# DavidPeicho/cuda-pathtracer

Measured on AMD Instinct MI355X. Metric: Msamples/sec at 1920x1080, 4 spp, indoor.obj, higher is better.
Workload: dtype f32

## Files before the change

### cuda-pathtracer_amd/csrc/pt_device.h

```cpp
#pragma once

#include <hip/hip_runtime.h>
#include <stdint.h>

#include "pt_round.h"

namespace ptamd {

struct f3 { float x, y, z; };

#define PT_DEV __device__ __forceinline__
#define PT_HD __host__ __device__ __forceinline__

PT_HD f3 mk3(float x, float y, float z) { f3 r; r.x = x; r.y = y; r.z = z; return r; }
PT_HD f3 mk3(float s) { return mk3(s, s, s); }
PT_HD f3 operator+(f3 a, f3 b) { return mk3(a.x + b.x, a.y + b.y, a.z + b.z); }
PT_HD f3 operator+(f3 a, float b) { return mk3(a.x + b, a.y + b, a.z + b); }
PT_HD f3 operator-(f3 a, f3 b) { return mk3(a.x - b.x, a.y - b.y, a.z - b.z); }
PT_HD f3 operator-(f3 a, float b) { return mk3(a.x - b, a.y - b, a.z - b); }
PT_HD f3 operator-(f3 a) { return mk3(-a.x, -a.y, -a.z); }
PT_HD f3 operator*(f3 a, f3 b) { return mk3(a.x * b.x, a.y * b.y, a.z * b.z); }
PT_HD f3 operator*(f3 a, float b) { return mk3(a.x * b, a.y * b, a.z * b); }
PT_HD f3 operator*(float b, f3 a) { return mk3(b * a.x, b * a.y, b * a.z); }
PT_HD f3 operator/(f3 a, f3 b) { return mk3(a.x / b.x, a.y / b.y, a.z / b.z); }
// ... 286 lines not shown
  while (!miss_tail_is_closed(thr)) {
    if (miss_tail_iteration(env, max_bounces, acc, thr, bk, r1, rng, rcp)) return futile;
    ++futile;
  }
  const f3 e = env * thr;
  const uint32_t n = miss_tail_count(bk & 0xffffu, max_bounces);
  for (uint32_t i = 0; i < n; ++i) acc = acc + e;
  return futile + n - 1u;
}


struct TexDesc { int32_t w, h, nb_chan; uint32_t pad; uint64_t offset; };

#define PT_HEAD_STRIDE 64u
#ifndef PT_TILE_W_LOG2
#define PT_TILE_W_LOG2 3u
#endif
#define PT_TILE_W (1u << PT_TILE_W_LOG2)
#define PT_TILE_H (64u >> PT_TILE_W_LOG2)
struct KParams {
  const float4* nodes;
  const float4* tris_bvh;
  const float4* tris_brute;
  const float4* shade;
  const int4* materials;
  const float4* lights;
  const TexDesc* textures;
  const float* texels;
  const float4* cubemap;
  uint32_t cubemap_size;
  uint32_t n_faces, n_lights, n_nodes, n_bvh_tris;
  f3 cam_pos, cam_p0, cam_u, cam_v;
  float focus_dist, aperture;
  uint32_t width, height, row_begin, row_end;
  uint32_t hash_seed;
  float frame_nb_f;
  float frame_nb_inv;
  int32_t is_static;
  int32_t bounces;
  uint32_t post_id;
  float* tfb;
  uint32_t* surface;
  uint32_t tfb_row0;
  uint32_t tfb_reset;
  uint32_t surf_row0;
  unsigned long long* stats;
  unsigned long long* error_flag;
  union { uint32_t* tile_counter; uint32_t* adaptive; };
  uint32_t* tile_heads;
  uint32_t n_static;
  uint32_t tiles_x, n_tiles, tiles_per_ticket;
  uint32_t refill_min;
  uint32_t sample_count, frame_nb0;
  float* samples_out;
  float4* pool;
  uint32_t pool_lds_offset;
  uint32_t round_min, round_div;
  uint32_t round_div_m16;
  uint32_t walk_min;
  uint32_t small_det;
  uint32_t env_uniform;
  float env_r, env_g, env_b;
  const float* gamma_table;
  const float4* nodes4;
  uint32_t n_nodes4;
  uint32_t stack_lds_entries, stack_spill_entries;
  uint32_t ilv_ranks, ilv_rank, ilv_rows;
  uint32_t y_limit;
  uint32_t treelet_nodes;
  uint2* stack_spill;
  uint32_t walk_min4;
  uint32_t wide8;
  uint32_t far_table[16];
  uint32_t xcd_regions;
  uint32_t brute_walk;
  unsigned long long* timeline;
  uint32_t round_form;
  uint32_t round_defer;
};
#define PT_ROUND_GENERIC 1u
#define PT_ROUND_FLAT 2u
#define PT_ROUND_SKIP 4u
#define PT_ROUND_DEFER 8u
#define PT_SKIP_ENTRY_BYTES 32u

#define PT_RS_PLAIN 0
#define PT_RS_STATS 1
#define PT_RS_STAMPS 2
#define PT_RS_BRUTE 3
#define PT_RS_WIDE8 4
#define PT_RS_WIDE4Q 5
#define PT_RS_GENERIC 6
#define PT_RS_LIST 7
#define PT_RS_FLAT 8
#define PT_RS_FLAT_SKIP 9
#define PT_RS_PLAIN_SKIP 10
#define PT_RS_FLAT_SKIP_DEFER 11
#define PT_RS_PLAIN_SKIP_DEFER 12
#define PT_RS_STATS_DEFER 13
#define PT_RS_FORMS 14

struct RestartTraits {
  bool stats;
  bool stamps;
  bool brute;
  int wide;
  bool list;
  bool lean;
  bool flat;
  bool skip;
  bool defer;
  int reports;
  bool resident, streamed, contracted;
};
constexpr RestartTraits kRestartForms[] = {
  { false, false, false, 0, false, true,  false, false, false, PT_RS_PLAIN,      true,  true,  true },
  { true,  false, false, 0, false, false, false, false, false, PT_RS_STATS,      true,  true,  false },
  { false, true,  false, 0, false, false, false, false, false, PT_RS_STAMPS,     true,  true,  false },
  { false, false, true,  0, false, false, false, false, false, PT_RS_BRUTE,      true,  true,  true },
  { false, false, false, 1, false, false, false, false, false, PT_RS_WIDE8,      false, true,  false },
  { false, false, false, 2, false, false, false, false, false, PT_RS_WIDE4Q,     false, true,  false },
  { false, false, false, 0, false, false, false, false, false, PT_RS_GENERIC,    true,  false, true },
  { false, false, false, 0, true,  false, false, false, false, PT_RS_LIST,       true,  true,  false },
  { false, false, false, 0, false, true,  true,  false, false, PT_RS_FLAT,       true,  false, false },
  { false, false, false, 0, false, true,  true,  true,  false, PT_RS_FLAT_SKIP,  true,  false, false },
  { false, false, false, 0, false, true,  false, true,  false, PT_RS_PLAIN_SKIP, true,  false, false },
  { false, false, false, 0, false, true,  true,  true,  true,  PT_RS_FLAT_SKIP,  true,  false, false },
  { false, false, false, 0, false, true,  false, true,  true,  PT_RS_PLAIN_SKIP, true,  false, false },
  { true,  false, false, 0, false, false, false, false, true,  PT_RS_STATS,      true,  false, false },
};
static_assert(sizeof kRestartForms / sizeof kRestartForms[0] == PT_RS_FORMS, "one row per PT_RS_* number");
constexpr RestartTraits restart_traits(int variant) { return kRestartForms[variant]; }

inline bool restart_shipped_launch(const KParams& p)
{
  return p.is_static && p.pool_lds_offset && !p.xcd_regions && p.ilv_ranks <= 1u && !(p.round_form & PT_ROUND_GENERIC);
}

struct RestartForm { int variant; bool lds_resident; };
inline RestartForm restart_select(bool lds_resident, bool stats, bool list, bool contracted, const KParams* p)
{
  const auto full = [contracted](int variant) { return contracted ? PT_RS_PLAIN : variant; };
  if (list && !contracted) return { PT_RS_LIST, lds_resident };
  const bool defers = p && lds_resident && !contracted && (p->round_form & PT_ROUND_DEFER) && (p->round_form & PT_ROUND_SKIP) && !p->brute_walk && !p->timeline &&
                      restart_shipped_launch(*p);
  if (stats) return { defers ? PT_RS_STATS_DEFER : full(PT_RS_STATS), lds_resident };
  if (p && p->brute_walk) return { PT_RS_BRUTE, lds_resident };
  if (p && p->timeline) return { full(PT_RS_STAMPS), lds_resident };
  if (!lds_resident && p && p->wide8) return { full(p->wide8 == 2u ? PT_RS_WIDE4Q : PT_RS_WIDE8), false };
  if (!lds_resident) return { PT_RS_PLAIN, false };
  if (p && !restart_shipped_launch(*p)) return { PT_RS_GENERIC, true };
  if (defers) return { (p->round_form & PT_ROUND_FLAT) ? PT_RS_FLAT_SKIP_DEFER : PT_RS_PLAIN_SKIP_DEFER, true };
  if (p && (p->round_form & PT_ROUND_SKIP) && !contracted) return { (p->round_form & PT_ROUND_FLAT) ? PT_RS_FLAT_SKIP : PT_RS_PLAIN_SKIP, true };
  if (p && (p->round_form & PT_ROUND_FLAT)) return { full(PT_RS_FLAT), true };
  return { PT_RS_PLAIN, true };
}
#define PT_POOL_LDS_BYTES 2304u

struct Hit {
  f3 normal;
  f3 diffuse_col;
  float dist;
  float specular_col;
  float ior;
  int light;
  float emission;
};

}
```

### cuda-pathtracer_amd/csrc/pt_kernels.hip

```cpp
#include "pt_device.h"
#include "pt_launch.h"
#include "pt_adaptive.h"

#include <utility>

#ifndef PT_FMA_BUILD
#include "pt_denoise.h"
#endif

namespace ptamd {

#ifndef PT_TILE_THREADS
#define PT_TILE_THREADS 512
#endif
#ifndef PT_TILE_WAVES_PER_EU
#define PT_TILE_WAVES_PER_EU 6
#endif
#ifndef PT_SP_THREADS
#define PT_SP_THREADS 768
#endif
#ifndef PT_SP_SHADERS
#define PT_SP_SHADERS 7
#endif
#ifndef PT_SP_WAVES_PER_EU
#define PT_SP_WAVES_PER_EU 6
#endif
#ifndef PT_SP_FETCH_MIN
#define PT_SP_FETCH_MIN 16u
#endif
#ifndef PT_BW_THREADS
#define PT_BW_THREADS 512
#endif
#ifndef PT_BW_WAVES_PER_EU
#define PT_BW_WAVES_PER_EU 4
#endif
#ifndef PT_BW_FETCH_MIN
#define PT_BW_FETCH_MIN 16u
#endif
#ifndef PT_PERSISTENT_WAVES_PER_EU
#define PT_PERSISTENT_WAVES_PER_EU 6
#endif
#ifndef PT_PERSISTENT_THREADS
#define PT_PERSISTENT_THREADS 512
#endif
#ifndef PT_RS_THREADS
#define PT_RS_THREADS 768
#endif
#ifndef PT_RS_WAVES_PER_EU
#define PT_RS_WAVES_PER_EU 6
#endif
#ifndef PT_ASM_LEAF
#define PT_ASM_LEAF 1
#endif
#ifndef PT_WALK_PRIO
#define PT_WALK_PRIO 3
#endif
#define PT_STR2(x) #x
#define PT_STR(x) PT_STR2(x)
#define PT_MAX_DIST 100000.0f
#define PT_END 0xFFFFFFFFu


struct Best { float t, u, v; uint32_t idx; };

template <bool ORDERED>
PT_DEV void mt_test(float4 a, float4 b, float4 c, f3 o, f3 d, Best& best, bool small_det = false)
{
  const f3 e1 = mk3(a.x, a.y, a.z);
  const f3 e2 = mk3(a.w, b.x, b.y);
  const f3 v0 = mk3(b.z, b.w, c.x);
  const f3 p_vec = cross(d, e2);
  const float det = dot(e1, p_vec);
  if (det < 1e-7f) return;
  const float inv_det = small_det ? rcp_exact_in_range(det) : 1.0f / det;
  const f3 t_vec = o - v0;
  const float u = dot(t_vec, p_vec) * inv_det;
  if (u < 0 || u > 1) return;
  const f3 qvec = cross(t_vec, e1);
  const float v = dot(d, qvec) * inv_det;
  if (v < 0 || u + v > 1) return;
  const float t = dot(e2, qvec) * inv_det;
  const uint32_t idx = f_as_u(c.y);
  bool take;
  if (ORDERED) take = t < best.t && t > 0.0f;
  else take = t > 0.0f && (t < best.t || (t == best.t && idx < best.idx && best.idx != PT_END));
  if (take) { best.t = t; best.u = u; best.v = v; best.idx = idx; }
}

PT_DEV void mt_test_asm(float4 a, float4 b, float2 c, f3 o, f3 d, Best& best)
// ... 160 lines not shown
                                       __builtin_fmaxf(t0z, t1z));
    const bool hit = tnear <= tfar && tfar >= 0.0f && tnear <= w.best.t;
    const uint32_t info = f_as_u(q0.w);
    const uint32_t child = f_as_u(q1.w);
    const uint32_t count = info >> 24;
    const uint32_t down = ((w.oct >> (child >> 30)) & 1u) ? (child & 0x3FFFFFFFu) : node + 1u;
    node = (hit && count == 0u) ? down : miss;
    if (hit && count != 0u) {
      leaf_first = info & 0xFFFFFFu;
      leaf_count = count;
      break;
    }
    if (walk_min > 1u && (uint32_t)__popcll(__ballot(1)) < walk_min) break;
  }
  w.node = node;
}

static_assert(PT_TILE_WAVES_PER_EU <= 6 && PT_PERSISTENT_WAVES_PER_EU <= 6 && PT_RS_WAVES_PER_EU <= 6 && PT_SP_WAVES_PER_EU <= 6,
              "walk_to_leaf_lds_state clobbers v64..v74: kernels that inline it need a budget of at least 75 VGPRs (<= 6 waves per SIMD)");
PT_DEV void walk_to_leaf_lds_state(uint32_t& state, uint32_t lnk, const Walk& w, uint32_t& leaf_first, uint32_t& leaf_count, uint32_t walk_min)
{
  unsigned long long save;
  uint32_t link_word;
  uint32_t walkers;
  asm volatile(
      "s_mov_b64 %[save], exec\n\t"
      "s_setprio " PT_STR(PT_WALK_PRIO) "\n\t"
      "v_cmp_gt_u32 vcc, 0x8000, %[st]\n\t"
      "s_and_b64 exec, exec, vcc\n\t"
      "s_cbranch_execz 2f\n\t"
      "1:\n\t"
      "v_add_u32 v74, %[st], %[lnk]\n\t"
      "ds_read_b128 v[64:67], %[st]\n\t"
      "ds_read_b64 v[68:69], %[st] offset:16\n\t"
      "ds_read_b32 %[lw], v74\n\t"
      "s_waitcnt lgkmcnt(1)\n\t"
      "v_fma_f32 v64, v64, %[ix], %[nx]\n\t"
      "v_fma_f32 v65, v65, %[iy], %[ny]\n\t"
      "v_fma_f32 v66, v66, %[iz], %[nz]\n\t"
      "v_fma_f32 v74, -v67, |%[ix]|, v64\n\t"
      "v_fma_f32 v64, v67, |%[ix]|, v64\n\t"
      "v_fma_f32 v67, -v68, |%[iy]|, v65\n\t"
      "v_fma_f32 v65, v68, |%[iy]|, v65\n\t"
      "v_fma_f32 v68, -v69, |%[iz]|, v66 clamp\n\t"
      "v_fma_f32 v66, v69, |%[iz]|, v66\n\t"
      "v_max3_f32 v74, v74, v67, v68\n\t"
      "v_min3_f32 v64, v64, v65, v66\n\t"
      "v_min_f32 v64, v64, %[best]\n\t"
      "v_cmp_le_f32 vcc, v74, v64\n\t"
      "s_waitcnt lgkmcnt(0)\n\t"
      "s_nop 0\n\t"
      "v_cndmask_b32_sdwa %[st], %[lw], %[lw], vcc dst_sel:DWORD dst_unused:UNUSED_PAD src0_sel:WORD_1 src1_sel:WORD_0\n\t"
      "v_cmpx_gt_u32 vcc, 0x8000, %[st]\n\t"
      "s_bcnt1_i32_b64 %[walkers], exec\n\t"
      "s_cmp_ge_u32 %[walkers], %[wmin]\n\t"
      "s_cbranch_scc1 1b\n\t"
      "2:\n\t"
      "s_mov_b64 exec, %[save]\n\t"
      "s_setprio 0\n\t"
      : [st] "+v"(state), [lw] "=&v"(link_word), [save] "=&s"(save), [walkers] "=&s"(walkers)
      : [wmin] "s"(walk_min), [lnk] "v"(lnk), [ix] "v"(w.inv.x), [iy] "v"(w.inv.y), [iz] "v"(w.inv.z),
        [nx] "v"(w.noi.x), [ny] "v"(w.noi.y), [nz] "v"(w.noi.z), [best] "v"(w.best.t * PT_T_SCALE)
      : "v64", "v65", "v66", "v67", "v68", "v69", "v74", "vcc", "scc", "memory");
  leaf_first = 0u;
  leaf_count = 0u;
  if (state >= 0x8000u && state != 0xFFFFu) {
    leaf_first = state & 0x7FFu;
    leaf_count = (state >> 11) & 0xFu;
    state = link_word >> 16;
  }
}

PT_DEV uint32_t walk_lds_link_offset(const Walk& w) { return w.n_nodes * 32u + w.oct * 4u; }
PT_DEV uint32_t walk_lds_state(uint32_t lds_nodes, uint32_t node) { return node == PT_END ? 0xFFFFu : lds_nodes + (node << 5); }
PT_DEV uint32_t walk_lds_node(uint32_t lds_nodes, uint32_t state) { return state == 0xFFFFu ? PT_END : (state - lds_nodes) >> 5; }

PT_DEV void walk_to_leaf_lds(uint32_t lds_nodes, Walk& w, uint32_t& leaf_first, uint32_t& leaf_count, uint32_t walk_min = 1u)
{
  uint32_t state = walk_lds_state(lds_nodes, w.node);
  walk_to_leaf_lds_state(state, walk_lds_link_offset(w), w, leaf_first, leaf_count, walk_min);
  w.node = walk_lds_node(lds_nodes, state);
}

template <bool STATS, bool ASM = false>
PT_DEV void walk_leaf(const float4* tris, Walk& w, uint32_t leaf_first, uint32_t leaf_count, uint32_t& n_tris,
                      uint32_t& wave_tri_iters, bool small_det = false, uint32_t stride = 3u )
{
  if (ASM && !STATS && PT_ASM_LEAF && small_det) {
    for (uint32_t k = 0; k < leaf_count; ++k) {
      const float4* r = tris + (leaf_first + k) * stride;
      const float4 a = r[0], b = r[1];
      const float2 c = *reinterpret_cast<const float2*>(r + 2);
      mt_test_asm(a, b, c, w.o, w.d, w.best);
    }
    return;
  }
  for (uint32_t k = 0; k < leaf_count; ++k) {
    if (STATS) {
      const unsigned long long act = __ballot(1);
      if ((threadIdx.x & 63u) == (uint32_t)(__ffsll((long long)act) - 1)) ++wave_tri_iters;
    }
    const uint32_t ti = (leaf_first + k) * stride;
    mt_test<false>(tris[ti], tris[ti + 1], tris[ti + 2], w.o, w.d, w.best, small_det);
  }
  if (STATS) n_tris += leaf_count;
}

template <bool STATS, bool NODES_IN_LDS = false>
PT_DEV void traverse_bvh(const float4* nodes, const float4* tris, uint32_t n_nodes, f3 o, f3 d,
                         Best& best, uint32_t& n_nodes_visited, uint32_t& n_tris, uint32_t& wave_node_iters,
                         uint32_t& wave_tri_iters, uint32_t* idle3)
{
  Walk w;
  walk_init(w, o, d, n_nodes, NODES_IN_LDS && !STATS);
  if (STATS) w.alive = (uint32_t)__popcll(__ballot(1));
  const uint32_t lds_nodes = (uint32_t)(uintptr_t)nodes;
  for (;;) {
    uint32_t leaf_first, leaf_count;
    if (NODES_IN_LDS && !STATS) walk_to_leaf_lds(lds_nodes, w, leaf_first, leaf_count);
    else walk_to_leaf<STATS>(nodes, w, leaf_first, leaf_count, n_nodes_visited, wave_node_iters);
    if (leaf_count != 0u) walk_leaf<STATS>(tris, w, leaf_first, leaf_count, n_tris, wave_tri_iters);
    else if (w.node == PT_END) break;
  }
  best = w.best;
  if (STATS) { idle3[0] += w.idle_unstarted; idle3[1] += w.idle_finished; idle3[2] += w.idle_parked; }
}

PT_DEV bool intersect_sphere(f3 o, f3 d, f3 center, float radius2 , float& t)
{
  const float epsilon = 0.01f;
  const f3 op = center - o;
  const float b = dot(op, d);
  float disc = b * b - dot(op, op) + radius2;
  if (disc < 0.0f) return false;
  disc = sqrt_checked(disc);
  t = b - disc;
  if (!(t > epsilon)) t = b + disc;
  return t != 0.0f;
}

PT_DEV int texture_idx(const TexDesc& tex, float uvx, float uvy)
{
  int x = (int)(uvx * (float)(tex.w - 1));
  int y = (int)(uvy * (float)(tex.h - 1));
  return (y * tex.w + x) * tex.nb_chan;
}

struct Counters { uint32_t rays, nodes, tris, mesh_hits, nmap_hits, wave_node_iters, wave_tri_iters, fetch_events, fetch_rays, idle3[3];
                  unsigned long long cyc[16]; };
#define PT_WAVE_ONE() ((threadIdx.x & 63u) == (uint32_t)(__ffsll((long long)__ballot(1)) - 1))

struct Nearest { float t, u, v; uint32_t idx; };
#define PT_LIGHT 0x80000000u

typedef const __attribute__((address_space(4))) float* ConstF;
PT_DEV ConstF as_constant(const float4* q) { return (ConstF)(uintptr_t)q; }

#define PT_KERNEL_PARAMS const KParams p
template <typename T>
PT_DEV T karg_load(uint32_t byte_offset)
{
  const __attribute__((address_space(4))) char* q = (const __attribute__((address_space(4))) char*)__builtin_amdgcn_kernarg_segment_ptr();
  asm volatile("" : "+s"(q));
  return *(const __attribute__((address_space(4))) T*)(q + byte_offset);
}
#define PT_KARG(p, field) karg_load<decltype(KParams::field)>((uint32_t)__builtin_offsetof(KParams, field))

PT_DEV Nearest nearest_lights(const KParams& p, f3 o, f3 d, Nearest n)
{
  const ConstF lights = as_constant(p.lights);
  for (uint32_t l = 0; l < p.n_lights; ++l) {
    const ConstF L = lights + l * 8u;
    const f3 c = mk3(L[3], L[4], L[5]);
    const f3 op = c - o;
    const float b = dot(op, d);
    const float disc = b * b - dot(op, op) + L[7];
    if (__builtin_amdgcn_ballot_w64(!(disc < 0.0f)) == 0ull) continue;
// ... 297 lines not shown
        const float f_t = 1.0f - f_r;
        st.throughput = st.throughput * (f_t * direct_light);
        st.o = st.o + oriented_normal * inter.dist / 10000.f;
        st.d = T;
      }
    }
  }
  if (STATS) { asm volatile("" : "+v"(st.d.x), "+v"(st.o.x), "+v"(st.throughput.x)); const long long tp1 = clock64(); if (PT_WAVE_ONE()) cnt.cyc[11] += (unsigned long long)(tp1 - tp0); }
  const float pmax = __builtin_fmaxf(st.throughput.x, __builtin_fmaxf(st.throughput.y, st.throughput.z));
  if (r1 > pmax && st.b() > 1u) return true;
  st.throughput = st.throughput * rcp_hot(pmax);
  ++st.bk;
  return (int)st.b() >= max_bounces;
}




PT_DEV void stage_to_lds(float4* dst, const float4* src, uint32_t n16)
{
  for (uint32_t i = threadIdx.x; i < n16; i += blockDim.x) dst[i] = src[i];
}

template <int KIND, bool STATS, bool NODES_IN_LDS = false>
PT_DEV bool path_step(const KParams& p, const float4* s_nodes, const float4* s_tris, Path& st, Counters& cnt)
{
  const float r1 = path_pre(p, st);
  const Nearest n = trace_nearest<KIND, STATS, NODES_IN_LDS>(p, s_nodes, s_tris, st.o, st.d, cnt);
  return path_post<STATS>(p, st, r1, n, cnt);
}


PT_DEV void path_finish(const KParams& p, const Path& st)
{
  f3 rad = mk3(clamp01(st.acc.x), clamp01(st.acc.y), clamp01(st.acc.z));
  const uint32_t x = st.x(), y = st.y();
  const size_t i = (size_t)(p.height - y - 1u - p.tfb_row0) * p.width + x;
  float* tp = p.tfb + i * 3;
  f3 t = p.tfb_reset ? mk3(0.0f) : mk3(tp[0], tp[1], tp[2]);
  t = t * (float)p.is_static;
  t = t + rad;
  tp[0] = t.x; tp[1] = t.y; tp[2] = t.z;
  rad = p.frame_nb_inv != 0.0f ? t * p.frame_nb_inv : t / p.frame_nb_f;
  rad = exposure(rad);
  uint32_t px;
  if (p.gamma_table && p.post_id == 0u) {
    px = gamma_byte(rad.x, p.gamma_table) | (gamma_byte(rad.y, p.gamma_table) << 8) | (gamma_byte(rad.z, p.gamma_table) << 16);
  } else {
    const float g = 1.0f / 2.2f;
    rad = mk3(pt_powf(rad.x, g), pt_powf(rad.y, g), pt_powf(rad.z, g));
    rad = post_process(p.post_id, rad);
    px = (pt_f2u(rad.x * 255.0f) & 0xffu) | ((pt_f2u(rad.y * 255.0f) & 0xffu) << 8) | ((pt_f2u(rad.z * 255.0f) & 0xffu) << 16);
  }
  p.surface[(size_t)(y - p.surf_row0) * p.width + x] = px;
}

PT_DEV void path_finish_sample(const KParams& p, const Path& st)
{
  const uint32_t row_begin = PT_KARG(p, row_begin), rows = PT_KARG(p, row_end) - row_begin;
  float* sp = PT_KARG(p, samples_out) + (((size_t)st.k() * rows + (st.y() - row_begin)) * PT_KARG(p, width) + st.x()) * 3;
  sp[0] = clamp01(st.acc.x); sp[1] = clamp01(st.acc.y); sp[2] = clamp01(st.acc.z);
}

template <bool STATS>
PT_DEV void flush_counters(const KParams& p, const Counters& cnt, uint32_t samples)
{
  if (!STATS) return;
  const uint32_t lane = threadIdx.x & 63u;
  unsigned long long v[13] = { cnt.rays, cnt.nodes, cnt.tris, cnt.mesh_hits, cnt.nmap_hits, samples,
                               cnt.wave_node_iters, cnt.wave_tri_iters, cnt.fetch_events, cnt.fetch_rays,
                               cnt.idle3[0], cnt.idle3[1], cnt.idle3[2] };
  for (int k = 0; k < 13; ++k) {
    unsigned long long s = v[k];
    for (int off = 32; off > 0; off >>= 1) s += __shfl_down(s, off, 64);
    if (lane == 0 && s) atomicAdd(&p.stats[k], s);
  }
  for (int k = 0; k < 16; ++k) {
    unsigned long long s = cnt.cyc[k];
    for (int off = 32; off > 0; off >>= 1) s += __shfl_down(s, off, 64);
    if (lane == 0 && s) atomicAdd(&p.stats[16 + k], s);
  }
}

template <int KIND, bool LDS_RESIDENT, bool COMPACT = false, bool SKIP = false>
PT_DEV void stage_scene(const KParams& p, float4* s_mem_, const float4*& s_nodes, const float4*& s_tris)
{
  float4* const s_mem = SKIP ? s_mem_ + PT_SKIP_ENTRY_BYTES / 16u : s_mem_;
  if (LDS_RESIDENT) {
    if (KIND == 1) {
      stage_to_lds(s_mem, p.tris_brute, p.n_faces * 3);
      s_nodes = nullptr;
      s_tris = s_mem;
    } else {
      if (COMPACT) {
        const uint32_t base = (uint32_t)(uintptr_t)s_mem;
        const uint32_t* relinked = reinterpret_cast<const uint32_t*>(p.nodes + p.n_nodes * 4);
        if (SKIP && threadIdx.x < 8u) {
          const uint32_t e = relinked[p.n_nodes * 8u + threadIdx.x];
          reinterpret_cast<uint32_t*>(s_mem_)[threadIdx.x] = e == 0xFFFFu ? PT_END : e;
        }
        if (base + p.n_nodes * 32u > 0x8000u || p.n_bvh_tris > 2047u) __builtin_trap();
        for (uint32_t i = threadIdx.x; i < p.n_nodes; i += blockDim.x) {
          const float4 q0 = p.nodes[i * 4 + 0], q1 = p.nodes[i * 4 + 1];
          const uint4 m0 = *reinterpret_cast<const uint4*>(p.nodes + i * 4 + 2), m1 = *reinterpret_cast<const uint4*>(p.nodes + i * 4 + 3);
          const uint32_t miss[8] = { m0.x, m0.y, m0.z, m0.w, m1.x, m1.y, m1.z, m1.w };
          const uint32_t child = f_as_u(q1.w), right = child & 0x3FFFFFFFu, axis = child >> 30;
          const bool leaf = (f_as_u(q0.w) >> 24) != 0u;
          uint32_t word[8];
          for (uint32_t o = 0; o < 8; ++o) {
            const uint32_t down = ((o >> axis) & 1u) ? right : i + 1u;
            const uint32_t ha = leaf ? (0x8000u | ((f_as_u(q0.w) >> 24) << 11) | (f_as_u(q0.w) & 0x7FFu)) : base + down * 32u;
            const uint32_t ma = miss[o] == PT_END ? 0xFFFFu : base + miss[o] * 32u;
            word[o] = ha | (ma << 16);
            if (SKIP) {
              const uint32_t w = relinked[i * 8u + o], hc = w & 0xFFFFu, mc = w >> 16;
              word[o] = (hc < 0x8000u ? base + hc * 32u : hc) | ((mc < 0x8000u ? base + mc * 32u : mc) << 16);
            }
          }
          float4* links = s_mem + p.n_nodes * 2u;
          float c[3], h[3];
          const float lo[3] = { q0.x, q0.y, q0.z }, hi[3] = { q1.x, q1.y, q1.z };
          for (int a = 0; a < 3; ++a) {
            c[a] = 0.5f * lo[a] + 0.5f * hi[a];
            h[a] = __builtin_fmaxf(hi[a] - c[a], c[a] - lo[a]) * 1.00000024f;
            if (!(__builtin_fabsf(lo[a]) <= 3.0e38f && __builtin_fabsf(hi[a]) <= 3.0e38f)) { c[a] = 0.0f; h[a] = 3.0e38f; }
          }
          s_mem[i * 2 + 0] = make_float4(c[0], c[1], c[2], h[0]);
          s_mem[i * 2 + 1] = make_float4(h[1], h[2], q0.w, 0.0f);
          links[i * 2 + 0] = make_float4(u_as_f(word[0]), u_as_f(word[1]), u_as_f(word[2]), u_as_f(word[3]));
          links[i * 2 + 1] = make_float4(u_as_f(word[4]), u_as_f(word[5]), u_as_f(word[6]), u_as_f(word[7]));
        }
      } else {
        stage_to_lds(s_mem, p.nodes, p.n_nodes * 4);
      }
      stage_to_lds(s_mem + p.n_nodes * 4, p.tris_bvh, p.n_bvh_tris * 3);
      s_nodes = s_mem;
      s_tris = s_mem + p.n_nodes * 4;
    }
    __syncthreads();
  } else {
    s_nodes = p.nodes;
    s_tris = KIND == 1 ? p.tris_brute : p.tris_bvh;
  }
}


template <int KIND, bool LDS_RESIDENT, bool STATS, int BLOCK>
__global__ void __launch_bounds__(BLOCK, PT_TILE_WAVES_PER_EU) pt_megakernel(PT_KERNEL_PARAMS)
{
  extern __shared__ float4 s_mem[];
  const float4* s_nodes;
  const float4* s_tris;
  stage_scene<KIND, LDS_RESIDENT, LDS_RESIDENT && !STATS>(p, s_mem, s_nodes, s_tris);

  const uint32_t lane = threadIdx.x & 63u, wave = threadIdx.x >> 6;
  const uint32_t x = blockIdx.x * 16u + (wave & 1u) * 8u + (lane & 7u);
  const uint32_t y = p.row_begin + blockIdx.y * (BLOCK / 16u) + (wave >> 1) * 8u + (lane >> 3);
  Counters cnt = {};
  const bool active = x < p.width && y < p.row_end;
  if (active) {
    Path st;
    path_begin(p, x, y, st);
    while (!path_step<KIND, STATS, LDS_RESIDENT>(p, s_nodes, s_tris, st, cnt)) {}
    path_finish(p, st);
  }
  flush_counters<STATS>(p, cnt, active ? 1u : 0u);
}


template <int KIND, bool LDS_RESIDENT, bool STATS>
__global__ void __launch_bounds__(PT_PERSISTENT_THREADS, PT_PERSISTENT_WAVES_PER_EU) pt_megakernel_persistent(PT_KERNEL_PARAMS)
{
  extern __shared__ float4 s_mem[];
  const float4* s_nodes;
  const float4* s_tris;
  stage_scene<KIND, LDS_RESIDENT, LDS_RESIDENT && !STATS>(p, s_mem, s_nodes, s_tris);

  const uint32_t lane = threadIdx.x & 63u;
  Counters cnt = {};
  uint32_t samples = 0;

  Path st;
// ... 87 lines not shown
}

PT_DEV void pool_load_lds(const uint32_t* pool, uint32_t e, Path& st)
{
  st.o = mk3(u_as_f(pool[e]), u_as_f(pool[64u + e]), u_as_f(pool[128u + e]));
  st.d = mk3(u_as_f(pool[192u + e]), u_as_f(pool[256u + e]), u_as_f(pool[320u + e]));
  st.rng.v2 = pool[384u + e]; st.rng.v3 = pool[448u + e]; st.rng.v4 = pool[512u + e];
  const uint32_t t1 = 2591861531u * 0xf7dcefddu;
  st.rng.v0 = 521288629u + t1;
  st.rng.v1 = 88675123u ^ t1;
  st.rng.d = 6615241u + t1 + (st.rng.v2 - 5783321u) + 2u * 362437u;
}

PT_DEV void pool_load(const float4* slab, uint32_t e, Path& st)
{
  typedef float v4f __attribute__((ext_vector_type(4)));
  const v4f* q = reinterpret_cast<const v4f*>(slab);
  const v4f a = __builtin_nontemporal_load(q + e);
  const v4f b = __builtin_nontemporal_load(q + 64u + e);
  const v4f c = __builtin_nontemporal_load(q + 128u + e);
  st.o = mk3(a.x, a.y, a.z);
  st.d = mk3(a.w, b.x, b.y);
  st.rng.v0 = f_as_u(b.z); st.rng.v1 = f_as_u(b.w);
  st.rng.v2 = f_as_u(c.x); st.rng.v3 = f_as_u(c.y); st.rng.v4 = f_as_u(c.z); st.rng.d = f_as_u(c.w);
}

template <bool STATS, bool NODES_IN_LDS>
PT_DEV void traverse_round_deferring(const float4* nodes, const float4* tris, uint32_t n_nodes, f3 o, f3 d, Best& best, uint32_t& node,
                                     uint32_t round_defer, uint32_t round_div, uint32_t round_div_m16, uint32_t walk_min, bool small_det, Counters& cnt)
{
  asm volatile("" : "+s"(round_defer));
  const uint32_t round_min = round_defer & 0xFFu;
  const uint32_t leaf_defer_knob = (round_defer >> 8) == 0xFFu ? PT_LEAF_DEFER_AUTO : round_defer >> 8;
  Walk w;
  walk_init(w, o, d, n_nodes, NODES_IN_LDS && !STATS);
  w.best = best;
  const uint32_t n_start = (uint32_t)__popcll(__ballot(node != PT_END));
  const uint32_t t_eff = round_threshold(n_start, round_min, round_div, round_div_m16);
  const uint32_t leaf_defer = round_leaf_defer(leaf_defer_knob, t_eff);
  uint32_t ctl = t_eff | ((leaf_defer < 255u ? leaf_defer : 255u) << 8) | 0x10000u;
  asm volatile("" : "+s"(ctl));
  if (STATS) w.alive = (uint32_t)__popcll(__ballot(1));
  const uint32_t lds_nodes = (uint32_t)(uintptr_t)nodes;
  if (NODES_IN_LDS && !STATS) {
    uint32_t state = round_is_pending(node) ? round_pending_leaf(node) : walk_lds_state(lds_nodes, node);
    const uint32_t lnk = walk_lds_link_offset(w);
    uint32_t leaf_first, leaf_count;
    for (;;) {
      const bool first = (ctl >> 16) != 0u;
      walk_to_leaf_lds_state(state, lnk, w, leaf_first, leaf_count, walk_min);
      if (first && round_is_pending(node)) state = round_pending_continuation(node);
      const uint32_t unfinished = (uint32_t)__popcll(__ballot(state != 0xFFFFu || leaf_count != 0u));
      if (!round_leaf_phase_runs(first, unfinished, (ctl >> 8) & 0xFFu)) break;
      if (leaf_count != 0u) walk_leaf<STATS, true>(tris, w, leaf_first, leaf_count, cnt.tris, cnt.wave_tri_iters, small_det);
      leaf_count = 0u;
      if (round_ends((uint32_t)__popcll(__ballot(state != 0xFFFFu)), ctl & 0xFFu)) break;
      ctl &= 0xFFFFu;
    }
    w.node = leaf_count != 0u ? round_pending_pack(0x8000u | (leaf_count << 11) | leaf_first, state) : walk_lds_node(lds_nodes, state);
  } else {
    w.node = round_is_pending(node) ? PT_END : node;
    for (;;) {
      const bool first = (ctl >> 16) != 0u;
      uint32_t leaf_first, leaf_count;
      walk_to_leaf<STATS>(nodes, w, leaf_first, leaf_count, cnt.nodes, cnt.wave_node_iters, walk_min);
      if (first && round_is_pending(node)) {
        leaf_first = round_pending_leaf(node) & 0x7FFu;
        leaf_count = (round_pending_leaf(node) >> 11) & 0xFu;
        w.node = round_pending_continuation(node) == 0xFFFFu ? PT_END : round_pending_continuation(node);
      }
      const uint32_t unfinished = (uint32_t)__popcll(__ballot(w.node != PT_END || leaf_count != 0u));
      if (!round_leaf_phase_runs(first, unfinished, (ctl >> 8) & 0xFFu)) {
        if (leaf_count != 0u) w.node = round_pending_pack(0x8000u | (leaf_count << 11) | leaf_first, w.node == PT_END ? 0xFFFFu : w.node);
        break;
      }
      if (leaf_count != 0u) walk_leaf<STATS>(tris, w, leaf_first, leaf_count, cnt.tris, cnt.wave_tri_iters, small_det);
      if (round_ends((uint32_t)__popcll(__ballot(w.node != PT_END)), ctl & 0xFFu)) break;
      ctl &= 0xFFFFu;
    }
  }
  best = w.best;
  node = w.node;
  if (STATS) { cnt.idle3[0] += w.idle_unstarted; cnt.idle3[1] += w.idle_finished; cnt.idle3[2] += w.idle_parked; }
}

template <bool STATS, bool NODES_IN_LDS, bool DEFER = false>
PT_DEV void traverse_round(const float4* nodes, const float4* tris, uint32_t n_nodes, f3 o, f3 d, Best& best, uint32_t& node,
                           uint32_t round_min, uint32_t round_div, uint32_t round_div_m16, uint32_t walk_min, bool small_det, Counters& cnt)
{
  if constexpr (DEFER) {
    traverse_round_deferring<STATS, NODES_IN_LDS>(nodes, tris, n_nodes, o, d, best, node, round_min, round_div, round_div_m16, walk_min, small_det, cnt);
    return;
  }
  Walk w;
  walk_init(w, o, d, n_nodes, NODES_IN_LDS && !STATS);
  w.best = best;
  w.node = node;
  const uint32_t n_start = (uint32_t)__popcll(__ballot(node != PT_END));
  uint32_t t_eff = ((n_start + round_div - 1u) * round_div_m16) >> 16;
  if (t_eff > round_min) t_eff = round_min;
  if (t_eff < 1u) t_eff = 1u;
  if (STATS) w.alive = (uint32_t)__popcll(__ballot(1));
  const uint32_t lds_nodes = (uint32_t)(uintptr_t)nodes;
  if (NODES_IN_LDS && !STATS) {
    uint32_t state = walk_lds_state(lds_nodes, w.node);
    const uint32_t lnk = walk_lds_link_offset(w);
    for (;;) {
      uint32_t leaf_first, leaf_count;
      walk_to_leaf_lds_state(state, lnk, w, leaf_first, leaf_count, walk_min);
      if (leaf_count != 0u) walk_leaf<STATS, true>(tris, w, leaf_first, leaf_count, cnt.tris, cnt.wave_tri_iters, small_det);
      if ((uint32_t)__popcll(__ballot(state != 0xFFFFu)) < t_eff) break;
    }
    w.node = walk_lds_node(lds_nodes, state);
  } else {
    for (;;) {
      uint32_t leaf_first, leaf_count;
      walk_to_leaf<STATS>(nodes, w, leaf_first, leaf_count, cnt.nodes, cnt.wave_node_iters, walk_min);
      if (leaf_count != 0u) walk_leaf<STATS>(tris, w, leaf_first, leaf_count, cnt.tris, cnt.wave_tri_iters, small_det);
      if ((uint32_t)__popcll(__ballot(w.node != PT_END)) < t_eff) break;
    }
  }
  best = w.best;
  node = w.node;
  if (STATS) { cnt.idle3[0] += w.idle_unstarted; cnt.idle3[1] += w.idle_finished; cnt.idle3[2] += w.idle_parked; }
}


#define PT_NONE 0xFFFFFFFFu
#define PT_LEAF_BIT 0x80000000u

struct Stack4 {
  uint2* lds;
  uint2* spill;
  uint32_t lds_entries;
  const float4* top;
  uint32_t top_n;
};
#ifndef PT_RS4_THREADS
#define PT_RS4_THREADS 1024
#endif
#define PT_TREELET_STRIDE 512u
static_assert(8u * PT_TREELET_STRIDE * 16u == kRestartTreeletRegionBytes, "lay_out_lds sizes the treelet's region: eight chunk planes of 16-byte words");
#ifndef PT_RS4_WAVES_PER_EU
#define PT_RS4_WAVES_PER_EU 4
#endif

typedef uint32_t pt_u2v __attribute__((ext_vector_type(2)));
typedef uint32_t pt_u4v __attribute__((ext_vector_type(4)));
typedef __attribute__((address_space(3))) pt_u2v* LdsU2;
typedef const __attribute__((address_space(3))) pt_u4v* LdsCU4;
PT_DEV LdsU2 stack4_lds(const Stack4& s) { return (LdsU2)(uintptr_t)(uint32_t)(uintptr_t)s.lds; }
PT_DEV LdsCU4 treelet_lds(const Stack4& s) { return (LdsCU4)(uintptr_t)(uint32_t)(uintptr_t)s.top; }
PT_DEV uint4 lds_u4(LdsCU4 q) { const pt_u4v v = *q; return make_uint4(v.x, v.y, v.z, v.w); }
PT_DEV float4 lds_f4(LdsCU4 q) { const pt_u4v v = *q; return make_float4(u_as_f(v.x), u_as_f(v.y), u_as_f(v.z), u_as_f(v.w)); }

PT_DEV void stack4_write(const Stack4& s, uint32_t k, uint32_t ref, float tnear)
{
  if (k < s.lds_entries) { pt_u2v e; e.x = ref; e.y = f_as_u(tnear); stack4_lds(s)[k * 64u] = e; }
  else s.spill[(size_t)(k - s.lds_entries) * 64u] = make_uint2(ref, f_as_u(tnear));
}

PT_DEV uint2 stack4_read(const Stack4& s, uint32_t k)
{
  if (k < s.lds_entries) { const pt_u2v e = stack4_lds(s)[k * 64u]; return make_uint2(e.x, e.y); }
  return s.spill[(size_t)(k - s.lds_entries) * 64u];
}
// ... 409 lines not shown
        else if (MODE == 2) cur = walk4q_visit<STATS>(nodes4, stk, w, x8.oct, cur, sp);
        else {
          long long tv0 = 0;
          if (STATS) tv0 = clock64();
          cur = walk4_visit<STATS>(nodes4, stk, w, cur, sp, &cnt);
          if (STATS) { const long long tv1 = clock64(); if (PT_WAVE_ONE()) cnt.cyc[7] += (unsigned long long)(tv1 - tv0); }
        }
      }
      if (walkers < walk_min) break;
    }
    long long tb1 = 0;
    if (STATS) {
      tb1 = clock64();
      const bool any_leaf = __ballot(cur != PT_NONE && (cur & PT_LEAF_BIT)) != 0ull;
      if (PT_WAVE_ONE()) { cnt.cyc[1] += (unsigned long long)(tb1 - tb0); if (any_leaf) cnt.cyc[5]++; }
    }
    if (cur != PT_NONE && (cur & PT_LEAF_BIT)) {
      const uint32_t first = cur & 0xFFFFFFu, count = (cur >> 24) & 0x7Fu;
      constexpr uint32_t TS = 3u;
      const float4* t = tris + (size_t)first * TS;
      float4 r[9];
#pragma unroll
      for (uint32_t k = 0; k < 3u; ++k)
        if (k < count) { r[3 * k] = t[TS * k]; r[3 * k + 1] = t[TS * k + 1]; r[3 * k + 2] = t[TS * k + 2]; }
#pragma unroll
      for (uint32_t k = 0; k < 3u; ++k)
        if (k < count) {
          if (STATS) {
            const unsigned long long act = __ballot(1);
            if ((threadIdx.x & 63u) == (uint32_t)(__ffsll((long long)act) - 1)) ++cnt.wave_tri_iters;
          }
          mt_test<false>(r[3 * k], r[3 * k + 1], r[3 * k + 2], w.o, w.d, w.best, small_det);
        }
      if (STATS) cnt.tris += count < 3u ? count : 3u;
      if (count > 3u) walk_leaf<STATS>(tris, w, first + 3u, count - 3u, cnt.tris, cnt.wave_tri_iters, small_det, TS);
      cur = stack4_pop4(stk, sp, w.best.t);
    }
    if (STATS && PT_WAVE_ONE()) cnt.cyc[2] += (unsigned long long)(clock64() - tb1);
    if ((uint32_t)__popcll(__ballot(cur != PT_NONE)) < t_eff) break;
  }
  best = w.best;
}

PT_DEV bool region_tile(const KParams& p, uint32_t ticket, uint32_t& col, uint32_t& row, uint32_t& k)
{
  const uint32_t r = ticket & 7u, i = ticket >> 3;
  const uint32_t tiles_x = PT_KARG(p, tiles_x), tiles_y = PT_KARG(p, n_tiles) / tiles_x, count = PT_KARG(p, sample_count);
  const uint32_t rx = r & 3u, ry = r >> 2;
  const uint32_t x0 = rx * tiles_x / 4u, x1 = (rx + 1u) * tiles_x / 4u, y0 = ry * tiles_y / 2u, y1 = (ry + 1u) * tiles_y / 2u;
  const uint32_t w = x1 - x0, h = y1 - y0;
  const uint32_t j = i / count;
  if (j >= w * h) return false;
  k = i - j * count;
  const uint32_t strips = w / 8u, full = strips * 8u * h;
  if (j < full) {
    const uint32_t s = j / (8u * h), rem = j - s * 8u * h;
    row = y0 + rem / 8u;
    col = x0 + s * 8u + (rem & 7u);
  } else {
    const uint32_t rem = j - full, wl = w - strips * 8u;
    row = y0 + rem / wl;
    col = x0 + strips * 8u + rem % wl;
  }
  return true;
}

#define PT_STAMP(slot)                                                                                                   \
  do {                                                                                                                   \
    if (FORM.stamps) {                                                                                                   \
      unsigned long long* tl_ = PT_KARG(p, timeline);                            \
      if ((threadIdx.x & 63u) == 0u)                                                                                     \
        tl_[(size_t)(blockIdx.x * (THREADS / 64u) + (threadIdx.x >> 6)) * 4u + (slot)] = wall_clock64();                 \
    }                                                                                                                    \
  } while (0)

template <bool LDS_RESIDENT, int VARIANT>
__global__ void __launch_bounds__(LDS_RESIDENT ? PT_RS_THREADS : PT_RS4_THREADS, LDS_RESIDENT ? PT_RS_WAVES_PER_EU : PT_RS4_WAVES_PER_EU)
pt_megakernel_restart(PT_KERNEL_PARAMS)
{
  constexpr RestartTraits FORM = restart_traits(VARIANT);
  constexpr bool STATS = FORM.stats;
  constexpr uint32_t THREADS = LDS_RESIDENT ? PT_RS_THREADS : PT_RS4_THREADS;
  constexpr bool DEFER = LDS_RESIDENT && FORM.defer;
  constexpr bool SKIP = LDS_RESIDENT && FORM.skip;
  constexpr bool FLAT = LDS_RESIDENT && FORM.flat;
  constexpr bool LEAN = LDS_RESIDENT && FORM.lean;
  constexpr bool LIST = FORM.list;
  constexpr bool FIXED = LEAN || LIST;
  extern __shared__ float4 s_mem[];
  const float4* s_nodes;
  const float4* s_tris;
  PT_STAMP(0);
  stage_scene<2, LDS_RESIDENT, LDS_RESIDENT && !STATS, SKIP>(p, s_mem, s_nodes, s_tris);
  constexpr bool WIDE = !LDS_RESIDENT;

  const uint32_t lane = threadIdx.x & 63u;
  const uint32_t gwave = blockIdx.x * (THREADS / 64u) + (threadIdx.x >> 6);
  float4* slab = p.pool + (size_t)gwave * 192u;
  uint32_t* lds_pool = reinterpret_cast<uint32_t*>(reinterpret_cast<char*>(s_mem) + p.pool_lds_offset) + (threadIdx.x >> 6) * 576u;
  Stack4 stk;
  stk.top = s_mem;
  stk.top_n = WIDE ? p.treelet_nodes : 0u;
  constexpr uint32_t NODE_F4 = FORM.wide == 2 ? 4u : 8u;
  const uint32_t treelet_f4 = (WIDE && p.treelet_nodes) ? 8u * PT_TREELET_STRIDE : 0u;
  if (WIDE) {
    constexpr uint32_t PLANE = PT_TREELET_STRIDE * (8u / NODE_F4);
    for (uint32_t i = threadIdx.x; i < p.treelet_nodes * NODE_F4; i += blockDim.x) s_mem[(i % NODE_F4) * PLANE + i / NODE_F4] = p.nodes4[i];
    __syncthreads();
  }
  PT_STAMP(1);
  stk.lds = reinterpret_cast<uint2*>(s_mem + (size_t)treelet_f4) + (size_t)(threadIdx.x >> 6) * p.stack_lds_entries * 64u + lane;
  stk.spill = p.stack_spill + (size_t)gwave * p.stack_spill_entries * 64u + lane;
  stk.lds_entries = p.stack_lds_entries;
  uint32_t cur = PT_NONE, sp = 0;
  Counters cnt = {};
  uint32_t samples = 0;

  Path st;
  st.o = st.d = st.throughput = st.acc = mk3(0.f);
  st.rng.v0 = st.rng.v1 = st.rng.v2 = st.rng.v3 = st.rng.v4 = st.rng.d = 0;
  st.specular_col = 0.f; st.xy = 0; st.bk = 0;
  bool idle = true;
  bool walking = false;
  Best best;
  best.t = PT_MAX_DIST; best.u = best.v = 0.f; best.idx = PT_END;
  uint32_t node = PT_END;
  uint32_t pool_rd = 64u, tile_x0 = 0, tile_y0 = 0, tile_k = 0;
  uint32_t tile_row_delta = 0;
  uint32_t tile = 0, tile_end = 0;
  uint32_t ticket = (!FIXED && PT_KARG(p, xcd_regions)) ? ((blockIdx.x >> 3) * (THREADS / 64u) + (threadIdx.x >> 6)) * 8u + (blockIdx.x & 7u) : gwave;
  ticket = (uint32_t)__builtin_amdgcn_readfirstlane((int)ticket);
  uint32_t reg_col = 0, reg_row = 0, reg_k = 0;
  uint32_t head = blockIdx.x & 7u, dry = 0;
  bool have_ticket = true, exhausted = false;
  uint32_t list_n = 0, list_chunks = 0, list_base = 0;
  if constexpr (LIST) {
    list_n = (uint32_t)__builtin_amdgcn_readfirstlane((int)*ad_active(p.adaptive, p.width * p.height));
    list_chunks = (list_n + 63u) >> 6;
  }
  for (;;) {
    long long tr0 = 0;
    if (STATS) tr0 = clock64();
    unsigned long long need = __ballot(idle);
    while (need) {
      if (pool_rd >= 64u) {
        if (exhausted) break;
        if (tile >= tile_end) {
          const uint32_t tiles_per_ticket = PT_KARG(p, tiles_per_ticket);
          uint32_t total;
          if constexpr (LIST) total = list_chunks * PT_KARG(p, sample_count);
          else total = PT_KARG(p, n_tiles) * PT_KARG(p, sample_count);
          for (;;) {
            if (!have_ticket) {
              uint32_t* heads = PT_KARG(p, tile_heads);
              uint32_t t = 0;
              if (lane == 0) t = atomicAdd(heads + head * PT_HEAD_STRIDE, 1u);
              t = (uint32_t)__builtin_amdgcn_readfirstlane((int)t);
              ticket = PT_KARG(p, n_static) + t * 8u + head;
            }
            have_ticket = false;
            if ((!FIXED && PT_KARG(p, xcd_regions)) ? region_tile(p, ticket, reg_col, reg_row, reg_k) : ((unsigned long long)ticket * tiles_per_ticket < total)) break;
            head = (head + 1u) & 7u;
            if (++dry == 8u) break;
          }
          if (dry == 8u) { exhausted = true; PT_STAMP(2); break; }
          if (!FIXED && PT_KARG(p, xcd_regions)) { tile = ticket; tile_end = ticket + 1u; }
          else {
            tile = ticket * tiles_per_ticket;
            tile_end = tile + tiles_per_ticket;
            if (tile_end > total) tile_end = total;
          }
        }
        if constexpr (LIST) {
          tile_k = tile / list_chunks;
          list_base = (tile - tile_k * list_chunks) * 64u;
        } else {
          const uint32_t n_tiles = PT_KARG(p, n_tiles), tiles_x = PT_KARG(p, tiles_x), row_begin = PT_KARG(p, row_begin);
          uint32_t local_y0;
          if (!FIXED && PT_KARG(p, xcd_regions)) {
            tile_k = reg_k; tile_x0 = reg_col * PT_TILE_W; local_y0 = reg_row * PT_TILE_H;
          } else {
            tile_k = tile / n_tiles;
            const uint32_t tl = tile - tile_k * n_tiles;
            tile_x0 = (tl % tiles_x) * PT_TILE_W;
            local_y0 = (tl / tiles_x) * PT_TILE_H;
          }
          const uint32_t ilv_ranks = LEAN ? 0u : PT_KARG(p, ilv_ranks);
          if (ilv_ranks > 1u) {
            const uint32_t ilv_rows = PT_KARG(p, ilv_rows);
            const uint32_t b = local_y0 / ilv_rows, within = local_y0 - b * ilv_rows;
            tile_y0 = (b * ilv_ranks + PT_KARG(p, ilv_rank)) * ilv_rows + within;
          } else {
            tile_y0 = row_begin + local_y0;
          }
          tile_row_delta = tile_y0 - (row_begin + local_y0);
        }
        ++tile;
        if constexpr (LIST) {
          const uint32_t i = list_base + lane;
          if (i < list_n) {
            const uint32_t n_px = p.width * p.height;
            const uint32_t px = ad_list(p.adaptive, n_px)[i];
            Path fresh;
            path_begin(p, px % p.width, px / p.width, fresh, tile_k, ad_counts(p.adaptive)[px] + 1u + tile_k);
            if (LDS_RESIDENT) pool_store_lds(lds_pool, lane, fresh);
            else pool_store(slab, lane, fresh);
          }
          if (!LDS_RESIDENT) asm volatile("s_waitcnt vmcnt(0)" ::: "memory");
        } else {
          const uint32_t x = tile_x0 + (lane & (PT_TILE_W - 1u)), y = tile_y0 + (lane >> PT_TILE_W_LOG2);
          if (x < p.width && y < p.y_limit) {
            Path fresh;
            path_begin(p, x, y, fresh, tile_k);
            if (LEAN || p.pool_lds_offset) pool_store_lds(lds_pool, lane, fresh);
            else pool_store(slab, lane, fresh);
          }
          if (!LEAN && !p.pool_lds_offset) asm volatile("s_waitcnt vmcnt(0)" ::: "memory");
        }
        pool_rd = 0u;
      }
      const uint32_t rank = __builtin_amdgcn_mbcnt_hi((uint32_t)(need >> 32), __builtin_amdgcn_mbcnt_lo((uint32_t)need, 0u));
      const uint32_t avail = 64u - pool_rd;
      if constexpr (LIST) {
        const uint32_t i = list_base + pool_rd + rank;
        if (idle && rank < avail && i < list_n) {
          if (LDS_RESIDENT) pool_load_lds(lds_pool, pool_rd + rank, st);
          else pool_load(slab, pool_rd + rank, st);
          st.throughput = mk3(1.0f);
          st.acc = mk3(0.0f);
          st.specular_col = 0.0f;
          st.xy = (i % p.width) | ((i / p.width) << 16);
          st.bk = tile_k << 16;
          idle = false;
          walking = false;
        }
      } else if (idle && rank < avail) {
        const uint32_t e = pool_rd + rank;
        const uint32_t x = tile_x0 + (e & (PT_TILE_W - 1u)), y = tile_y0 + (e >> PT_TILE_W_LOG2);
        if (x < p.width && y < p.y_limit) {
          if (LEAN || p.pool_lds_offset) pool_load_lds(lds_pool, e, st);
          else pool_load(slab, e, st);
          st.throughput = mk3(1.0f);
          st.acc = mk3(0.0f);
          st.specular_col = 0.0f;
          st.xy = x | ((y - tile_row_delta) << 16);
          st.bk = tile_k << 16;
          idle = false;
          walking = false;
        }
      }
      const uint32_t wanted = (uint32_t)__popcll(need);
      pool_rd += wanted < avail ? wanted : avail;
      need = __ballot(idle);
    }
    if (__ballot(!idle) == 0ull) break;
    long long tr1 = 0;
    if (STATS) { tr1 = clock64(); if (PT_WAVE_ONE()) cnt.cyc[0] += (unsigned long long)(tr1 - tr0); }

    if (!idle) {
      if (!walking) {
        best.t = PT_MAX_DIST; best.u = 0.f; best.v = 0.f; best.idx = PT_END;
        if (SKIP) node = reinterpret_cast<const uint32_t*>(s_mem)[(st.d.x < 0.f ? 1u : 0u) | (st.d.y < 0.f ? 2u : 0u) | (st.d.z < 0.f ? 4u : 0u)];
        else node = p.n_nodes ? 0u : PT_END;
        cur = p.n_nodes4 ? 0u : PT_NONE;
        sp = 0u;
        walking = true;
        if (STATS) cnt.rays++;
      }
      if (FORM.brute) {
        for (uint32_t i = 0; i < p.n_bvh_tris; ++i) mt_test<false>(s_tris[i * 3u], s_tris[i * 3u + 1u], s_tris[i * 3u + 2u], st.o, st.d, best, false);
        if (STATS) cnt.tris += p.n_bvh_tris;
        node = PT_END;
      } else if (WIDE) {
        traverse_round4<STATS, FORM.wide>(p, p.nodes4, s_tris, stk, st.o, st.d, best, cur, sp, p.round_min, p.round_div, p.round_div_m16, p.walk_min4, p.small_det != 0u, cnt);
        node = cur == PT_NONE ? PT_END : 0u;
      } else {
        traverse_round<STATS, LDS_RESIDENT, DEFER>(s_nodes, s_tris, p.n_nodes, st.o, st.d, best, node, DEFER ? p.round_defer : p.round_min, p.round_div, p.round_div_m16, p.walk_min, p.small_det != 0u, cnt);
      }
      if (STATS) {
        if (lane == (uint32_t)(__ffsll((long long)__ballot(1)) - 1)) cnt.fetch_events++;
        if (node == PT_END) cnt.fetch_rays++;
      }
      if (node == PT_END) {
        long long tl0 = 0;
        if (STATS) tl0 = clock64();
        const float r1 = path_pre<FIXED>(p, st);
        Nearest n;
        n.t = best.t; n.u = best.u; n.v = best.v; n.idx = best.idx;
        n = nearest_lights(p, st.o, st.d, n);
        walking = false;
        long long tl1 = 0;
        if (STATS) { asm volatile("" : "+v"(n.t), "+v"(n.idx)); tl1 = clock64(); if (PT_WAVE_ONE()) cnt.cyc[3] += (unsigned long long)(tl1 - tl0); }
        if (path_post<STATS, FIXED, FLAT>(p, st, r1, n, cnt)) {
          path_finish_sample(p, st);
          idle = true;
          if (STATS) samples++;
        }
        if (STATS) { const long long tl2 = clock64(); if (PT_WAVE_ONE()) cnt.cyc[9] += (unsigned long long)(tl2 - tl1); }
      }
    }
    if (STATS) {
      const long long tr3 = clock64();
      if (PT_WAVE_ONE()) cnt.cyc[4] += (unsigned long long)(tr3 - tr0);
    }
  }
  PT_STAMP(3);
  flush_counters<STATS>(p, cnt, samples);
}


template <bool LDS_RESIDENT, bool STATS>
__global__ void __launch_bounds__(PT_BW_THREADS, PT_BW_WAVES_PER_EU) pt_megakernel_blockwise(PT_KERNEL_PARAMS)
{
  constexpr uint32_t NW = PT_BW_THREADS / 64u;
  constexpr uint32_t NE = NW * 8u;
  constexpr uint32_t EPL = (NE + 63u) / 64u;
  static_assert(NW % 4u == 0 && NE <= 128u, "workgroup must be 4k waves, at most 16");
  extern __shared__ float4 s_mem[];
  const float4* s_nodes;
  const float4* s_tris;
  stage_scene<2, LDS_RESIDENT>(p, s_mem, s_nodes, s_tris);
  float4* pool = s_mem + (LDS_RESIDENT ? (p.n_nodes * 4u + p.n_bvh_tris * 3u) : 0u);
  uint32_t* s_cnt = reinterpret_cast<uint32_t*>(pool + PT_BW_THREADS * 2u);
  uint32_t* s_head = s_cnt + 128;
  uint32_t* s_ticket = s_cnt + 129;

  const uint32_t tid = threadIdx.x, lane = tid & 63u, wave = tid >> 6;
  Counters cnt = {};
  uint32_t samples = 0;
  uint32_t ticket = blockIdx.x;

  for (;;) {
    if (ticket >= p.n_tiles) break;
    const uint32_t sx = (ticket % p.tiles_x) * 32u, sy = p.row_begin + (ticket / p.tiles_x) * (NW * 2u);
    const uint32_t x = sx + (wave & 3u) * 8u + (lane & 7u);
    const uint32_t y = sy + (wave >> 2) * 8u + (lane >> 3);
    const bool active = x < p.width && y < p.row_end;
    Path st;
    bool live = active;
    if (active) path_begin(p, x, y, st);
    else { st.o = st.d = st.throughput = st.acc = mk3(0.f); st.xy = 0; st.bk = 0; st.specular_col = 0.f;
           st.rng.v0 = st.rng.v1 = st.rng.v2 = st.rng.v3 = st.rng.v4 = st.rng.d = 0; }

    if (live) live = !path_step<2, STATS>(p, s_nodes, s_tris, st, cnt);

    for (;;) {
      const uint32_t oct = (st.d.x < 0.f ? 1u : 0u) | (st.d.y < 0.f ? 2u : 0u) | (st.d.z < 0.f ? 4u : 0u);
      uint32_t rank = 0, my_count = 0;
#pragma unroll
      for (uint32_t o = 0; o < 8u; ++o) {
        const unsigned long long m = __ballot(live && oct == o);
        const uint32_t c = (uint32_t)__popcll(m);
        if (oct == o) rank = __builtin_amdgcn_mbcnt_hi((uint32_t)(m >> 32), __builtin_amdgcn_mbcnt_lo((uint32_t)m, 0u));
        if (lane == o) my_count = c;
      }
      if (lane < 8u) s_cnt[lane * NW + wave] = my_count;
      if (tid == 0) *s_head = 0u;
      __syncthreads();
      uint32_t e0 = 0, e1 = 0;
      if (lane * EPL < NE) e0 = s_cnt[lane * EPL];
      if (EPL == 2u && lane * EPL + 1u < NE) e1 = s_cnt[lane * EPL + 1u];
      uint32_t incl = e0 + e1;
#pragma unroll
      for (int off = 1; off < 64; off <<= 1) {
        const uint32_t up = __shfl_up(incl, off, 64);
        if ((int)lane >= off) incl += up;
// ... 356 lines not shown
  stk.top = s_mem;
  stk.top_n = p.treelet_nodes;
  stk.lds = reinterpret_cast<uint2*>(s_mem + (p.treelet_nodes ? 8u * PLANE_NODES : 0u)) + (size_t)(threadIdx.x >> 6) * p.stack_lds_entries * 64u + lane;
  stk.spill = p.stack_spill + (size_t)gwave * p.stack_spill_entries * 64u + lane;
  stk.lds_entries = p.stack_lds_entries;
  Counters cnt = {};
  Walk w;
  walk_init(w, mk3(0.f), mk3(0.f, 0.f, 1.f), 1u);
  uint32_t cur = PT_NONE, sp = 0u, ray = PT_NONE;
  uint32_t chunk_next = 0u, chunk_end = 0u;
  bool exhausted = false;
  const bool small_det = false;
  for (;;) {
    const unsigned long long idle = __ballot(ray == PT_NONE);
    const uint32_t n_idle = (uint32_t)__popcll(idle);
    if (!exhausted && n_idle != 0u && (n_idle >= p.refill_min || n_idle == 64u)) {
      if (chunk_next >= chunk_end) {
        uint32_t base = 0u;
        if (lane == 0u) base = atomicAdd(head, 512u);
        chunk_next = (uint32_t)__builtin_amdgcn_readfirstlane((int)base);
        chunk_end = chunk_next + 512u < n ? chunk_next + 512u : n;
        if (chunk_next >= n) { exhausted = true; chunk_next = chunk_end = n; }
      }
      const uint32_t rank = __builtin_amdgcn_mbcnt_hi((uint32_t)(idle >> 32), __builtin_amdgcn_mbcnt_lo((uint32_t)idle, 0u));
      if (ray == PT_NONE && chunk_next + rank < chunk_end) {
        ray = chunk_next + rank;
        const float* r = rays + (size_t)ray * 6u;
        walk_init(w, mk3(r[3], r[4], r[5]), mk3(r[0], r[1], r[2]), 1u);
        cur = p.n_nodes4 ? 0u : PT_NONE;
        sp = 0u;
      }
      chunk_next = chunk_next + n_idle < chunk_end ? chunk_next + n_idle : chunk_end;
    }
    if (__ballot(ray != PT_NONE) == 0ull) break;
    if (ray != PT_NONE) {
      w.oct_x = __ballot((w.oct & 1u) != 0u); w.oct_y = __ballot((w.oct & 2u) != 0u); w.oct_z = __ballot((w.oct & 4u) != 0u);
      for (;;) {
        const bool interior = cur < PT_LEAF_BIT;
        const uint32_t walkers = (uint32_t)__popcll(__ballot(interior));
        if (walkers == 0u) break;
        if (interior) cur = walk4_visit<false, PLANE_BYTES>(p.nodes4, stk, w, cur, sp);
        if (walkers < p.walk_min4) break;
      }
      if (cur != PT_NONE && (cur & PT_LEAF_BIT)) {
        const uint32_t first = cur & 0xFFFFFFu, count = (cur >> 24) & 0x7Fu;
        const float4* t = p.tris_bvh + (size_t)first * 3u;
        float4 r[9];
#pragma unroll
        for (uint32_t k = 0; k < 3u; ++k)
          if (k < count) { r[3 * k] = t[3 * k]; r[3 * k + 1] = t[3 * k + 1]; r[3 * k + 2] = t[3 * k + 2]; }
#pragma unroll
        for (uint32_t k = 0; k < 3u; ++k)
          if (k < count) mt_test<false>(r[3 * k], r[3 * k + 1], r[3 * k + 2], w.o, w.d, w.best, small_det);
        if (count > 3u) walk_leaf<false>(p.tris_bvh, w, first + 3u, count - 3u, cnt.tris, cnt.wave_tri_iters, small_det);
        cur = stack4_pop4(stk, sp, w.best.t);
      }
      if (cur == PT_NONE) {
        Nearest nr;
        nr.t = w.best.t; nr.u = w.best.u; nr.v = w.best.v; nr.idx = w.best.idx;
        nr = nearest_lights(p, w.o, w.d, nr);
        const int kind = nr.idx == PT_END ? 0 : ((nr.idx & PT_LIGHT) ? 2 : 1);
        const int index = kind == 0 ? -1 : (int)(nr.idx & ~PT_LIGHT);
        out[ray] = make_int4(kind, index, (int)f_as_u(nr.t), 0);
        ray = PT_NONE;
      }
    }
  }
}

template <int KIND>
__global__ void __launch_bounds__(256) pt_trace_rays_kernel(PT_KERNEL_PARAMS, const float* rays, uint32_t n, int4* out)
{
  const uint32_t i = blockIdx.x * blockDim.x + threadIdx.x;
  if (i >= n) return;
  const f3 d = mk3(rays[i * 6 + 0], rays[i * 6 + 1], rays[i * 6 + 2]);
  const f3 o = mk3(rays[i * 6 + 3], rays[i * 6 + 4], rays[i * 6 + 5]);
  Counters cnt = {};
  const Nearest nr = trace_nearest<KIND, false>(p, p.nodes, KIND == 1 ? p.tris_brute : p.tris_bvh, o, d, cnt);
  const int kind = nr.idx == PT_END ? 0 : ((nr.idx & PT_LIGHT) ? 2 : 1);
  const int index = kind == 0 ? -1 : (int)(nr.idx & ~PT_LIGHT);
  out[i] = make_int4(kind, index, (int)f_as_u(nr.t), 0);
}

#ifndef PT_FMA_BUILD

template <int KIND>
__global__ void __launch_bounds__(256) pt_features_kernel(PT_KERNEL_PARAMS, float4* feat, float* rays)
{
  const uint32_t x = blockIdx.x * 16u + (threadIdx.x & 15u), y = blockIdx.y * 16u + (threadIdx.x >> 4);
  if (x >= p.width || y >= p.height) return;
  const int half_w = (int)(p.width / 2u), half_h = (int)(p.height / 2u);
  const f3 screen_pos = (p.cam_p0 + (p.cam_u * (float)((int)x - half_w))) + (p.cam_v * (float)((int)y - half_h));
  const f3 dir = normalize_hot(screen_pos - p.cam_pos);
  const f3 d = normalize_hot(p.focus_dist * dir);
  const f3 o = p.cam_pos;
  Counters cnt = {};
  const Nearest n = trace_nearest<KIND, false>(p, p.nodes, KIND == 1 ? p.tris_brute : p.tris_bvh, o, d, cnt);
  Hit hit;
  hit.normal = mk3(0.f); hit.diffuse_col = mk3(0.f);
  hit.dist = 0.f; hit.specular_col = 0.f; hit.ior = 0.f; hit.light = -1; hit.emission = 0.f;
  const bool found = resolve_hit<false>(p, d, n, hit, cnt);
  const uint32_t kind = !found ? PT_FEAT_MISS : ((n.idx & PT_LIGHT) ? PT_FEAT_LIGHT : PT_FEAT_MESH);
  const uint32_t index = kind == PT_FEAT_MISS ? PT_FEAT_NO_INDEX : (n.idx & ~PT_LIGHT);
  const f3 albedo = found ? hit.diffuse_col : env_lookup(p, d);
  const f3 nrm = found ? hit.normal : mk3(0.f);
  const size_t i = (size_t)y * p.width + x;
  feat[2 * i] = make_float4(nrm.x, nrm.y, nrm.z, n.t);
  feat[2 * i + 1] = make_float4(albedo.x, albedo.y, albedo.z, u_as_f(kind << 30 | index));
  if (rays) {
    float* r = rays + i * 6;
    r[0] = d.x; r[1] = d.y; r[2] = d.z; r[3] = o.x; r[4] = o.y; r[5] = o.z;
  }
}

template <int PASS>
__global__ void __launch_bounds__(256) pt_denoise_kernel(const DenoiseParams q)
{
  const uint32_t x = blockIdx.x * 16u + (threadIdx.x & 15u), y = blockIdx.y * 16u + (threadIdx.x >> 4);
  if (x >= q.width || y >= q.height) return;
  if (PASS == 0) dn_prepare(q, x, y);
  else if (PASS == 1) dn_variance(q, x, y);
  else if (PASS == 2) dn_level(q, x, y);
  else dn_plain(q, x, y);
}

hipError_t launch_features(const KParams& p, int kind, float4* feat_dev, float* rays_dev, hipStream_t stream)
{
  const dim3 grid((p.width + 15u) / 16u, (p.height + 15u) / 16u);
  if (kind == 1) hipLaunchKernelGGL(pt_features_kernel<1>, grid, dim3(256), 0, stream, p, feat_dev, rays_dev);
  else hipLaunchKernelGGL(pt_features_kernel<2>, grid, dim3(256), 0, stream, p, feat_dev, rays_dev);
  return hipGetLastError();
}

hipError_t launch_denoise_pass(const DenoiseParams& q, int pass, hipStream_t stream)
{
  const dim3 grid((q.width + 15u) / 16u, (q.height + 15u) / 16u);
  switch (pass) {
  case 0: hipLaunchKernelGGL(pt_denoise_kernel<0>, grid, dim3(256), 0, stream, q); break;
  case 1: hipLaunchKernelGGL(pt_denoise_kernel<1>, grid, dim3(256), 0, stream, q); break;
  case 2: hipLaunchKernelGGL(pt_denoise_kernel<2>, grid, dim3(256), 0, stream, q); break;
  default: hipLaunchKernelGGL(pt_denoise_kernel<3>, grid, dim3(256), 0, stream, q); break;
  }
  return hipGetLastError();
}
#endif


#define PT_FN(...) reinterpret_cast<const void*>(__VA_ARGS__)
#ifndef PT_FMA_BUILD
static const void* const kTileEntries[2][2][2] = {
  { { PT_FN(pt_megakernel<1, false, false, PT_TILE_THREADS>), PT_FN(pt_megakernel<1, false, true, PT_TILE_THREADS>) },
    { PT_FN(pt_megakernel<1, true, false, PT_TILE_THREADS>), PT_FN(pt_megakernel<1, true, true, PT_TILE_THREADS>) } },
  { { PT_FN(pt_megakernel<2, false, false, PT_TILE_THREADS>), PT_FN(pt_megakernel<2, false, true, PT_TILE_THREADS>) },
    { PT_FN(pt_megakernel<2, true, false, PT_TILE_THREADS>), PT_FN(pt_megakernel<2, true, true, PT_TILE_THREADS>) } } };
static const void* const kPersistentEntries[2][2] = {
  { PT_FN(pt_megakernel_persistent<2, false, false>), PT_FN(pt_megakernel_persistent<2, false, true>) },
  { PT_FN(pt_megakernel_persistent<2, true, false>), PT_FN(pt_megakernel_persistent<2, true, true>) } };
static const void* const kSplitEntries[2][2] = {
  { PT_FN(pt_megakernel_split<false, false>), PT_FN(pt_megakernel_split<false, true>) },
  { PT_FN(pt_megakernel_split<true, false>), PT_FN(pt_megakernel_split<true, true>) } };
static const void* const kBlockwiseEntries[2][2] = {
  { PT_FN(pt_megakernel_blockwise<false, false>), PT_FN(pt_megakernel_blockwise<false, true>) },
  { PT_FN(pt_megakernel_blockwise<true, false>), PT_FN(pt_megakernel_blockwise<true, true>) } };
constexpr bool kContracted = false;
#else
constexpr bool kContracted = true;
#endif

template <int V>
static const void* restart_entry_of(bool lds_resident)
{
  constexpr RestartTraits FORM = restart_traits(V);
  if constexpr (FORM.contracted || !kContracted) {
    if constexpr (FORM.resident) { if (lds_resident) return PT_FN(pt_megakernel_restart<true, V>); }
    if constexpr (FORM.streamed) { if (!lds_resident) return PT_FN(pt_megakernel_restart<false, V>); }
  }
  return nullptr;
}
template <int... V>
static const void* restart_entry_among(std::integer_sequence<int, V...>, int variant, bool lds_resident)
{
  const void* fn = nullptr;
  ((variant == V ? void(fn = restart_entry_of<V>(lds_resident)) : void()), ...);
  return fn;
}
static const void* restart_entry(int variant, bool lds_resident)
{
  return restart_entry_among(std::make_integer_sequence<int, PT_RS_FORMS>(), variant, lds_resident);
}

uint32_t restart_threads(bool lds_resident) { return lds_resident ? PT_RS_THREADS : PT_RS4_THREADS; }
uint32_t restart_wide_blocks_per_cu() { return (PT_RS4_WAVES_PER_EU * 256u) / PT_RS4_THREADS; }

static KernelForm restart_form(bool lds_resident, bool stats, bool list, size_t lds_bytes, const KParams* p)
{
  const RestartForm launched = restart_select(lds_resident, stats, list, kContracted, p);
  const RestartForm queried = restart_select(lds_resident, false, list, kContracted, nullptr);
  const uint32_t threads = restart_threads(lds_resident);
  KernelForm f = { restart_entry(launched.variant, launched.lds_resident), restart_entry(queried.variant, queried.lds_resident), threads,
                   threads / 64u, lds_bytes, kFormSlotRestart, "restart", launched.variant };
  if (kContracted) { f.cache_slot = kFormSlotRestartContracted; f.name = "contracted restart"; }
  else if (list) { f.cache_slot = kFormSlotRestartList; f.name = "restart (list form)"; }
  return f;
}

#ifndef PT_FMA_BUILD
KernelForm megakernel_form(uint32_t kernel, bool lds_resident, bool stats, bool list, size_t lds_bytes, const KParams* p)
{
  const int r = lds_resident ? 1 : 0, s = stats ? 1 : 0;
  const size_t scene = lds_resident ? lds_bytes : 0;
  switch (kernel) {
    case PTAMD_KERNEL_BRUTE_FORCE:
    case PTAMD_KERNEL_BVH: {
      const void* fn = kTileEntries[kernel == PTAMD_KERNEL_BVH ? 1 : 0][r][s];
      return { fn, fn, PT_TILE_THREADS, 0u, scene, kFormSlotTile, "tile" };
    }
    case PTAMD_KERNEL_BVH_PERSISTENT:
      return { kPersistentEntries[r][s], kPersistentEntries[r][0], PT_PERSISTENT_THREADS, PT_PERSISTENT_THREADS / 64u, scene, kFormSlotPersistent, "persistent" };
    case PTAMD_KERNEL_BVH_BLOCKWISE:
      return { kBlockwiseEntries[r][s], kBlockwiseEntries[r][0], PT_BW_THREADS, 1u, scene + (size_t)PT_BW_THREADS * 32u + 128u * 4u + 16u, kFormSlotBlockwise, "blockwise" };
    case PTAMD_KERNEL_BVH_SPLIT:
      return { kSplitEntries[r][s], kSplitEntries[r][0], PT_SP_THREADS, PT_SP_SHADERS, scene + (size_t)PT_SP_SHADERS * 64u * 32u + (2u * PT_SP_SHADERS + 4u) * 4u, kFormSlotSplit, "split" };
    case PTAMD_KERNEL_BVH_RESTART_FMA: {
      KernelForm f;
      ptamd_fma_restart_form(r, lds_bytes, p, &f);
      return f;
    }
    default: return restart_form(lds_resident, stats, list, lds_bytes, p);
  }
}

static hipError_t allow_lds(const void* fn, size_t lds_bytes)
{
  return lds_bytes > 64 * 1024 ? hipFuncSetAttribute(fn, hipFuncAttributeMaxDynamicSharedMemorySize, (int)lds_bytes) : hipSuccess;
}

hipError_t form_blocks_per_cu(const KernelForm& f, int* out)
{
  const hipError_t e = allow_lds(f.occupancy_fn, f.lds_bytes);
  return e != hipSuccess ? e : hipOccupancyMaxActiveBlocksPerMultiprocessor(out, f.occupancy_fn, (int)f.threads, f.lds_bytes);
}

hipError_t launch_form(const KernelForm& f, const KParams& p, uint32_t n_blocks, hipStream_t stream)
{
  if (!f.fn) return hipErrorInvalidDeviceFunction;
  dim3 grid(n_blocks);
  if (f.ticket_waves == 0u) {
    const uint32_t rows = p.row_end - p.row_begin, block_rows = f.threads / 16u;
    grid = dim3((p.width + 15u) / 16u, (rows + block_rows - 1u) / block_rows);
  } else if (p.n_tiles == 0) return hipSuccess;
  if (grid.x == 0 || grid.y == 0) return hipSuccess;
  const hipError_t e = allow_lds(f.fn, f.lds_bytes);
  if (e != hipSuccess) return e;
  KParams pc = p;
  void* args[] = { &pc };
  return hipLaunchKernel(f.fn, grid, dim3(f.threads), args, f.lds_bytes, stream);
}

hipError_t launch_resolve(const KParams& p, hipStream_t stream)
{
  const uint32_t n = (p.row_end - p.row_begin) * p.width;
  if (n == 0) return hipSuccess;
  const bool wide = (p.width % 4u) == 0u && ((uintptr_t)p.tfb % 16u) == 0u && ((uintptr_t)p.samples_out % 16u) == 0u &&
                    ((uintptr_t)p.surface % 16u) == 0u;
  if (wide) hipLaunchKernelGGL(pt_resolve_kernel4, dim3((n / 4u + 255u) / 256u), dim3(256), 0, stream, p);
  else hipLaunchKernelGGL(pt_resolve_kernel, dim3((n + 255u) / 256u), dim3(256), 0, stream, p);
  return hipGetLastError();
}

hipError_t build_gamma_table(float* table_dev, hipStream_t stream)
{
  hipLaunchKernelGGL(pt_build_gamma_table, dim3(1), dim3(320), 0, stream, table_dev);
  return hipGetLastError();
}

hipError_t launch_gamma_selftest(const float* table_dev, uint32_t first, uint32_t count, unsigned long long* out_dev, hipStream_t stream)
{
  if (count == 0) return hipSuccess;
  hipLaunchKernelGGL(pt_gamma_selftest, dim3(4096), dim3(256), 0, stream, table_dev, first, count, out_dev);
  return hipGetLastError();
}

hipError_t resolve_kernels()
{
  hipError_t e = hipSuccess;
  const auto resolve = [&e](const void* const* fns, size_t n) {
    hipFuncAttributes attr;
    for (size_t i = 0; i < n && e == hipSuccess; ++i) e = hipFuncGetAttributes(&attr, fns[i]);
  };
  resolve(&kTileEntries[0][0][0], 8);
  resolve(&kPersistentEntries[0][0], 4);
  resolve(&kSplitEntries[0][0], 4);
  resolve(&kBlockwiseEntries[0][0], 4);
  for (int variant = 0; variant < PT_RS_FORMS; ++variant)
    for (int r = 0; r < 2; ++r) if (const void* fn = restart_entry(variant, r != 0)) resolve(&fn, 1);
  const void* const others[] = {
    PT_FN(pt_resolve_kernel), PT_FN(pt_resolve_kernel4), PT_FN(pt_trace_rays_kernel<1>), PT_FN(pt_trace_rays_kernel<2>),
    PT_FN(pt_trace_rays_wide_kernel<0>), PT_FN(pt_trace_rays_wide_kernel<1>), PT_FN(pt_trace_rays_wide_kernel<2>),
    PT_FN(pt_features_kernel<1>), PT_FN(pt_features_kernel<2>),
    PT_FN(pt_denoise_kernel<0>), PT_FN(pt_denoise_kernel<1>), PT_FN(pt_denoise_kernel<2>), PT_FN(pt_denoise_kernel<3>),
  };
  resolve(others, sizeof others / sizeof others[0]);
  return e;
}

static const void* trace_queue_entry(uint32_t config, uint32_t* threads, uint32_t* plane_nodes, uint32_t* blocks_per_cu)
{
  switch (config) {
    case 1: *threads = 640; *plane_nodes = 256; *blocks_per_cu = 2; return reinterpret_cast<const void*>(pt_trace_queue_kernel<640, 5, 256>);
    case 2: *threads = 768; *plane_nodes = 256; *blocks_per_cu = 2; return reinterpret_cast<const void*>(pt_trace_queue_kernel<768, 6, 256>);
    case 3: *threads = 1024; *plane_nodes = 256; *blocks_per_cu = 1; return reinterpret_cast<const void*>(pt_trace_queue_kernel<1024, 4, 256>);
    default: *threads = 1024; *plane_nodes = 512; *blocks_per_cu = 1; return reinterpret_cast<const void*>(pt_trace_queue_kernel<1024, 4, 512>);
  }
}

void trace_queue_shape(uint32_t config, uint32_t* threads, uint32_t* plane_nodes, uint32_t* blocks_per_cu)
{
  (void)trace_queue_entry(config, threads, plane_nodes, blocks_per_cu);
}

hipError_t launch_trace_queue(const KParams& p, uint32_t config, size_t lds_bytes, uint32_t n_blocks, const float* rays_dev, uint32_t n, int4* out_dev,
                              uint32_t* head_dev, int* resident_blocks_per_cu, hipStream_t stream)
{
  uint32_t threads, plane, bpc;
  const void* fn = trace_queue_entry(config, &threads, &plane, &bpc);
  if (resident_blocks_per_cu && lds_bytes > 64 * 1024) {
    hipError_t e = hipFuncSetAttribute(fn, hipFuncAttributeMaxDynamicSharedMemorySize, (int)lds_bytes);
    if (e != hipSuccess) return e;
  }
  if (resident_blocks_per_cu) {
    hipError_t e = hipOccupancyMaxActiveBlocksPerMultiprocessor(resident_blocks_per_cu, fn, (int)threads, lds_bytes);
    if (e != hipSuccess) return e;
  }
  KParams pc = p;
  void* args[] = { &pc, &rays_dev, &n, &out_dev, &head_dev };
  return hipLaunchKernel(fn, dim3(n_blocks), dim3(threads), args, lds_bytes, stream);
}

hipError_t launch_trace_rays(const KParams& p, int kind, const float* rays_dev, uint32_t n, int4* out_dev,
                             hipStream_t stream)
{
  if (n == 0) return hipSuccess;
  if (kind == 3) {
    const size_t lds = (size_t)p.stack_lds_entries * 64u * sizeof(uint2);
    const void* fn = p.wide8 == 1u ? PT_FN(pt_trace_rays_wide_kernel<1>) : (p.wide8 == 2u ? PT_FN(pt_trace_rays_wide_kernel<2>) : PT_FN(pt_trace_rays_wide_kernel<0>));
    const hipError_t e = allow_lds(fn, lds);
    if (e != hipSuccess) return e;
    KParams pc = p;
    void* args[] = { &pc, &rays_dev, &n, &out_dev };
    return hipLaunchKernel(fn, dim3((n + 63u) / 64u), dim3(64), args, lds, stream);
  }
  dim3 grid((n + 255u) / 256u);
  if (kind == 1) hipLaunchKernelGGL(pt_trace_rays_kernel<1>, grid, dim3(256), 0, stream, p, rays_dev, n, out_dev);
  else hipLaunchKernelGGL(pt_trace_rays_kernel<2>, grid, dim3(256), 0, stream, p, rays_dev, n, out_dev);
  return hipGetLastError();
}

#else
}
extern "C" void ptamd_fma_restart_form(int lds_resident, size_t lds_bytes, const ptamd_fma::KParams* p, ptamd_fma::KernelForm* out)
{
  *out = ptamd::restart_form(lds_resident != 0, false, false, lds_bytes, p);
}
namespace ptamd {
#endif
}
```

### cuda-pathtracer_amd/csrc/pt_launch.h

```cpp
#pragma once

#include <hip/hip_runtime.h>
#include <stdint.h>

#include "ptamd.h"

namespace ptamd {

struct KParams;
struct DenoiseParams;
struct TemporalParams;

struct KernelForm {
  const void* fn;
  const void* occupancy_fn;
  uint32_t threads;
  uint32_t ticket_waves;
  size_t lds_bytes;
  uint32_t cache_slot;
  const char* name;
  int restart_form = -1;
};
enum : uint32_t { kFormSlotTile, kFormSlotPersistent, kFormSlotBlockwise, kFormSlotSplit, kFormSlotRestart, kFormSlotRestartContracted, kFormSlotRestartList, kFormSlots };
KernelForm megakernel_form(uint32_t kernel, bool lds_resident, bool stats, bool list, size_t lds_bytes, const KParams* p);
hipError_t form_blocks_per_cu(const KernelForm& f, int* out);
hipError_t launch_form(const KernelForm& f, const KParams& p, uint32_t n_blocks, hipStream_t stream);
uint32_t restart_threads(bool lds_resident);
constexpr uint32_t kRestartTreeletRegionBytes = 64u * 1024u;
uint32_t restart_wide_blocks_per_cu();
hipError_t launch_resolve(const KParams& p, hipStream_t stream);
hipError_t build_gamma_table(float* table_dev, hipStream_t stream);
hipError_t launch_gamma_selftest(const float* table_dev, uint32_t first, uint32_t count, unsigned long long* out_dev, hipStream_t stream);
hipError_t resolve_kernels();
void trace_queue_shape(uint32_t config, uint32_t* threads, uint32_t* plane_nodes, uint32_t* blocks_per_cu);
hipError_t launch_trace_queue(const KParams& p, uint32_t config, size_t lds_bytes, uint32_t n_blocks, const float* rays_dev, uint32_t n, int4* out_dev,
                              uint32_t* head_dev, int* resident_blocks_per_cu, hipStream_t stream);
hipError_t launch_trace_rays(const KParams& p, int kind, const float* rays_dev, uint32_t n, int4* out_dev,
                             hipStream_t stream);
hipError_t launch_features(const KParams& p, int kind, float4* feat_dev, float* rays_dev, hipStream_t stream);
hipError_t launch_denoise_pass(const DenoiseParams& q, int pass, hipStream_t stream);
struct AdaptiveParams;
hipError_t launch_adaptive_select(const AdaptiveParams& a, hipStream_t stream);
hipError_t launch_adaptive_resolve_list(const AdaptiveParams& a, hipStream_t stream);
hipError_t launch_adaptive_resolve(const AdaptiveParams& a, hipStream_t stream);
hipError_t launch_temporal_pass(const DenoiseParams& q, const TemporalParams& t, int pass, hipStream_t stream);
struct MotionParams;
hipError_t launch_motion_reproject(const DenoiseParams& q, const TemporalParams& t, const MotionParams& m, hipStream_t stream);

}

extern "C" void ptamd_fma_restart_form(int lds_resident, size_t lds_bytes, const ptamd::KParams* p, ptamd::KernelForm* out);
```

### cuda-pathtracer_amd/csrc/ptamd_host.h

```cpp
#pragma once

#include "../host/ptamd_internal.h"
#include "pt_device.h"
#include "pt_launch.h"
#include "pt_refit.h"
#include "ptamd_owners.h"
#include "ptamd_tuning.h"

#include <string>
#include <type_traits>
#include <vector>

namespace ptamd {

struct DeviceScene {
  DeviceBuffer<float4> nodes;
  DeviceBuffer<float4> nodes4;
  DeviceBuffer<float4> nodes8;
  DeviceBuffer<float4> nodes4q;
  uint32_t n_nodes8 = 0, depth8 = 0;
  DeviceBuffer<float4> tris_bvh;
  DeviceBuffer<float4> tris_brute;
  DeviceBuffer<float4> shade;
  bool flat = false;
  DeviceBuffer<int4> materials;
  DeviceBuffer<float4> lights;
  DeviceBuffer<TexDesc> textures;
  DeviceBuffer<float> texels;
  uint32_t n_faces = 0, n_lights = 0, n_nodes = 0, n_materials = 0, n_textures = 0;
  uint32_t n_bvh_tris = 0;
  uint32_t n_nodes4 = 0, depth4 = 0;
  float extent = 0.0f;
  bool all_finite = true;
  uint32_t n_skipped = 0;
  bool links = false, cull_on = false;
  uint32_t n_culled = 0;
  DeviceBuffer<uint32_t> links_plain;
  Bvh topology;
  std::vector<uint32_t> record_face;
  std::vector<uint8_t> skip_set, cull_bits;
  std::vector<uint32_t> link_words;
  PinnedBuffer<uint32_t> h_links[2];
  float reach = 0.0f;
  float margin_floor = 0.0f;
  ptamd_scene_info info{};
  bool released = false;
  bool refit_ok = false;
  std::vector<uint32_t> material_ids;
  std::vector<ptamd_light> host_lights;
  DeviceBuffer<float> raw;
  DeviceBuffer<uint32_t> refit_groups;
  DeviceBuffer<uint32_t> refit_levels;
  DeviceBuffer<uint32_t> refit_sched;
  DeviceBuffer<uint32_t> wide_child;
  uint32_t n_refit_groups = 0, n_refit_levels = 0, n_refit_sched = 0, refit_top_first = 0, refit_top_levels = 0;
  DeviceBuffer<float> d_faces;
  PinnedBuffer<ptamd_face> h_stage[2];
  Event staged[2];
  bool staged_valid[2] = { false, false };
  uint32_t stage_next = 0;
  Event updated;
  bool updated_valid = false;
  uint64_t geometry_serial = 0;
  DeviceBuffer<float> d_margin;
  PinnedBuffer<float> h_margin;
  Event margin_ready[2];
  bool margin_ready_valid[2] = { false, false };
  uint32_t margin_next = 0, margin_slot = 0;
  bool margins_pending = false;
  PinnedBuffer<ptamd_light> h_lights[2];
  Event lights_staged[2];
  bool lights_staged_valid[2] = { false, false };
  uint32_t lights_next = 0;
  double quality_built = 0.0;
  DeviceBuffer<double> d_quality;
};

struct DeviceCubemap {
  DeviceBuffer<float4> faces;
  uint32_t size = 0;
  bool uniform = false;
  float color[3] = { 0.f, 0.f, 0.f };
};

}

struct ptamd_context {
  int device = 0;
  ptamd::TuningSettings knobs;
  std::vector<ptamd::DeviceScene> scenes;
  std::vector<ptamd::DeviceCubemap> cubemaps;
  uint32_t frame_counter = 0;
  bool last_restart_deferred = false;
  int32_t last_restart_form = -1;
  ptamd::DeviceBuffer<unsigned long long> d_stats;
  ptamd::DeviceBuffer<float> d_gamma;
  ptamd::DeviceBuffer<uint32_t> d_tickets;
  ptamd::DeviceBuffer<uint32_t> d_heads;
  uint32_t ticket_next = 0;
  std::vector<bool> heads_clean;
  std::vector<bool> slot_pinned;
  int n_cus = 0;
  struct Occupancy { size_t lds = ~(size_t)0; int blocks_per_cu = -1; } occupancy[ptamd::kFormSlots];
  struct SampleScratch {
    void* stream = nullptr;
    ptamd::DeviceBuffer<float> buf[4];
    size_t bytes[4] = { 0, 0, 0, 0 };
    ptamd::Event mega_done[3];
    ptamd::Event resolved[3];
    bool resolved_valid[3] = { false, false, false };
    ptamd::Event last_done;
    uint32_t flip = 0;
    bool no_pipeline = false;
    bool captured = false;
    std::vector<uint32_t> pinned_slots;
  };
  std::vector<SampleScratch> sample_scratch;
  static constexpr uint32_t kMaxLanes = 4;
  ptamd::Stream lane[kMaxLanes];
  uint32_t n_lanes = 0;
  ptamd::Stream internal[2];
  uint32_t lane_next = 0;
  ptamd::DeviceBuffer<uint2> d_trace_spill;
  struct { uint32_t config = ~0u; size_t lds = 0; int resident = 0; } trace_queue_cache;
  size_t trace_spill_bytes = 0;
  ptamd::DeviceBuffer<unsigned long long> d_timeline;
  uint32_t timeline_waves = 0;
  ptamd::DeviceBuffer<float4> d_denoise;
  size_t denoise_pixels = 0;
};

static_assert(!std::is_copy_constructible<ptamd::DeviceScene>::value && !std::is_copy_constructible<ptamd::DeviceCubemap>::value &&
              !std::is_copy_constructible<ptamd_context::SampleScratch>::value && !std::is_copy_constructible<ptamd_context>::value,
              "structs that own device resources move, they are never copied");

namespace ptamd {

constexpr size_t kLdsBudget = 64 * 1024;
constexpr uint32_t kCompactMaxNodes = 896;
constexpr uint32_t kCompactMaxTris = 2047;
constexpr float kBoxMargin = 1e-3f;
constexpr uint32_t kTicketRing = 1024;
constexpr uint32_t kMaxFramesPerSlab = 4;

int hip_fail(const char* what, hipError_t e);

#define PT_HIP(call)                                         \
  do {                                                       \
    hipError_t _e = (call);                                  \
    if (_e != hipSuccess) return hip_fail(#call, _e);        \
  } while (0)

inline bool live_scene(const ptamd_context* ctx, uint32_t scene_id)
{
  return scene_id < ctx->scenes.size() && !ctx->scenes[scene_id].released;
}

int bring_up(ptamd_context* ctx, hipStream_t s);
bool stream_is_capturing(hipStream_t stream);

bool far_origin_camera(const DeviceScene& s, const ptamd_camera& cam);
int settle_margins(DeviceScene& s, hipStream_t stream, const char* who);
void fill_scene(const DeviceScene& s, const DeviceCubemap* cm, KParams& p);
int wait_for_update(const DeviceScene& s, hipStream_t stream, bool capturing);
int update_scene_checks(const char* who, const ptamd_context* ctx, uint32_t scene_id, uint32_t n_faces, const void* faces);
int update_capture_checks(const char* who, const ptamd_context* ctx, hipStream_t stream);
int wait_for_readers(const ptamd_context* ctx, const DeviceScene& s, hipStream_t stream);
int device_array_checks(const char* who, const char* what, const ptamd_context* ctx, const void* p, size_t bytes, bool aligned16);
int prepare_device_refit(const char* who, DeviceScene& s, RefitParams& r);
int enqueue_device_refit(DeviceScene& s, RefitParams& r, const float* faces, hipStream_t stream);

float frame_nb_inverse(float c);
float camera_terms(const ptamd_camera& cam, uint32_t width, KParams& p);
int do_launch(ptamd_context* ctx, const ptamd_launch* l, bool stats, const AdaptiveParams* ad = nullptr);

}
// ... 1 lines not shown
```

### cuda-pathtracer_amd/csrc/ptamd_launch.cpp

```cpp
#include "ptamd_host.h"
#include "pt_adaptive.h"

#include <algorithm>
#include <cmath>
#include <cstdlib>
#include <cstring>

namespace ptamd {

float frame_nb_inverse(float c)
{
  uint32_t bits;
  std::memcpy(&bits, &c, 4);
  const uint32_t exponent = bits >> 23;
  if ((bits & 0x007FFFFFu) != 0u || exponent < 1u || exponent > 253u) return 0.0f;
  return 1.0f / c;
}

namespace {

constexpr float kQuantisedMaxExtent = 1.0e8f;
constexpr size_t kMaxScratchStreams = 16;

void fill_far_table(uint32_t t[16])
// ... 90 lines not shown
}

uint32_t choose_wide_nodes(const ptamd_context* ctx, const DeviceScene& s, bool knobs, KParams& p)
{
  const bool quantised_ok = knobs && s.extent <= kQuantisedMaxExtent;
  if (quantised_ok && ctx->knobs.wide8 && s.n_nodes8 != 0) {
    p.nodes4 = s.nodes8.get(); p.n_nodes4 = s.n_nodes8; p.wide8 = 1u;
    return 7u * s.depth8 + 1u;
  }
  if (quantised_ok && ctx->knobs.wide4q && s.nodes4q) { p.nodes4 = s.nodes4q.get(); p.wide8 = 2u; }
  return 3u * s.depth4 + 1u;
}

struct LaunchPlan {
  uint32_t which = 0;
  bool fma = false;
  bool brute_walk = false;
  bool resident = false;
  size_t lds = 0, launch_lds = 0;
  hipStream_t stream = nullptr;
  ptamd_context::SampleScratch* sc = nullptr;
  bool capturing = false, pipelined = false;
  uint32_t waves_per_block = 0, n_blocks = 0, slab = 3, slot = 0;
};

inline bool persistent_family(uint32_t k) { return k == PTAMD_KERNEL_BVH_PERSISTENT || k == PTAMD_KERNEL_BVH_SPLIT || k == PTAMD_KERNEL_BVH_RESTART; }

int resolve_kernel(const ptamd_context* ctx, const ptamd_launch* l, bool stats, const AdaptiveParams* ad, LaunchPlan& pl)
{
  pl.fma = l->kernel == PTAMD_KERNEL_BVH_RESTART_FMA;
  if (pl.fma && stats) { set_error("ptamd_raytrace_stats: the contracted kernel has no instrumented build"); return PTAMD_ERR_ARG; }
  pl.which = pl.fma ? (uint32_t)PTAMD_KERNEL_BVH_RESTART : l->kernel;
  if (pl.which == PTAMD_KERNEL_AUTO) pl.which = ad ? (uint32_t)PTAMD_KERNEL_BVH_RESTART : ctx->knobs.default_kernel;
  const DeviceScene& s = ctx->scenes[l->scene_id];
  const bool far_origin = far_origin_camera(s, l->camera);
  if (far_origin) {
    if (pl.which == PTAMD_KERNEL_BVH_RESTART) pl.brute_walk = true;
    else pl.which = PTAMD_KERNEL_BRUTE_FORCE;
  }
  if (l->interleave_ranks > 1u && pl.which != PTAMD_KERNEL_BVH_RESTART) {
    set_error("ptamd_raytrace: interleaved bands need the restart kernel (PTAMD_KERNEL_AUTO resolves to another one here)");
    return PTAMD_ERR_ARG;
  }
  if (l->frame_count > 1 && !far_origin && !persistent_family(pl.which)) {
    set_error("ptamd_raytrace: frame_count > 1 needs a persistent kernel (PTAMD_KERNEL_AUTO, _BVH_PERSISTENT, _BVH_RESTART or _BVH_SPLIT)");
    return PTAMD_ERR_ARG;
  }
  const bool brute = pl.which == PTAMD_KERNEL_BRUTE_FORCE;
  pl.lds = pl.launch_lds = brute ? s.info.lds_bytes_brute : s.info.lds_bytes_bvh;
  pl.resident = pl.lds <= kLdsBudget && (brute || (s.n_nodes <= kCompactMaxNodes && s.n_bvh_tris <= kCompactMaxTris));
  pl.stream = static_cast<hipStream_t>(l->stream);
  return PTAMD_OK;
}

void fill_launch(const ptamd_context* ctx, const ptamd_launch* l, bool stats, const LaunchPlan& pl, KParams& p)
{
  const DeviceScene& s = ctx->scenes[l->scene_id];
  std::memset(&p, 0, sizeof p);
  fill_scene(s, &ctx->cubemaps[l->cubemap_id], p);
  p.gamma_table = ctx->d_gamma.get();
  fill_far_table(p.far_table);
  p.small_det = ctx->knobs.short_rcp && s.all_finite && s.extent <= 1.0e8f ? 1u : 0u;
  camera_terms(l->camera, l->width, p);
  p.width = l->width; p.height = l->height; p.row_begin = l->row_begin; p.row_end = l->row_end;
  p.hash_seed = ptamd_wang_hash(l->frame_nb);
  p.frame_nb_f = (float)(int)l->frame_nb;
  p.frame_nb_inv = frame_nb_inverse(p.frame_nb_f);
  p.is_static = l->moved ? 0 : 1;
  p.bounces = (int32_t)l->bounces;
  p.post_id = l->post_id;
  p.tfb = l->temporal_framebuffer;
  p.tfb_reset = l->reset_accumulation ? 1u : 0u;
  p.surface = static_cast<uint32_t*>(l->surface_rgba8);
  if (l->band_local_buffers) {
    p.tfb_row0 = l->height - l->row_end;
    p.surf_row0 = l->row_begin;
  }
  p.stats = stats ? ctx->d_stats.get() : nullptr;
  p.error_flag = ctx->d_stats.get() + 15;
  p.brute_walk = pl.brute_walk ? 1u : 0u;
  p.round_form = (ctx->knobs.generic_round ? PT_ROUND_GENERIC : 0u) | (ctx->knobs.flat_round && s.flat && ctx->cubemaps[l->cubemap_id].uniform ? PT_ROUND_FLAT : 0u);
  const bool defer = ctx->knobs.leaf_defer != 0u && (ctx->knobs.leaf_defer != PT_LEAF_DEFER_AUTO || (p.round_form & PT_ROUND_FLAT));
  if (s.links && pl.resident) p.round_form |= PT_ROUND_SKIP | (defer ? PT_ROUND_DEFER : 0u);
}

int plan_stream(ptamd_context* ctx, const ptamd_launch* l, bool stats, bool later_chunk, const AdaptiveParams* ad, LaunchPlan& pl)
{
  for (auto& c : ctx->sample_scratch) if (c.stream == l->stream) pl.sc = &c;
  if (!pl.sc) {
    if (ctx->sample_scratch.size() >= kMaxScratchStreams) {
      size_t pinned = 0;
      for (auto& c : ctx->sample_scratch) pinned += c.captured ? 1u : 0u;
      if (pinned >= kMaxScratchStreams) {
        set_error("ptamd_raytrace: all 16 per-stream sample scratches of this context are pinned by captured graphs (ptamd_release_captured)");
        return PTAMD_ERR_LIMIT;
      }
      PT_HIP(hipDeviceSynchronize());
      std::vector<ptamd_context::SampleScratch> kept;
      for (auto& c : ctx->sample_scratch) if (c.captured) kept.push_back(std::move(c));
      ctx->sample_scratch.swap(kept);
    }
    ctx->sample_scratch.emplace_back();
    pl.sc = &ctx->sample_scratch.back();
    pl.sc->stream = l->stream;
  }
  pl.pipelined = ctx->knobs.overlap && pl.which == PTAMD_KERNEL_BVH_RESTART && !stats && !ad;
  if (stream_is_capturing(pl.stream)) pl.capturing = true;
  if (pl.capturing || pl.sc->no_pipeline || l->no_pipelining) pl.pipelined = false;
  if (pl.pipelined && !later_chunk)
    pl.pipelined = pl.sc->last_done && (l->machine_share > 1u || hipEventQuery(pl.sc->last_done.get()) == hipErrorNotReady);
  if (pl.pipelined && pl.stream != nullptr) {
    const uint32_t want = l->machine_share >= 3u ? ptamd_context::kMaxLanes : 2u;
    while (ctx->n_lanes < want) { int rc = add_lane(ctx); if (rc != PTAMD_OK) return rc; }
  }
  if (l->kernel == PTAMD_KERNEL_AUTO && pl.which == PTAMD_KERNEL_BVH_RESTART && ctx->knobs.default_kernel_is_builtin && l->frame_count <= 1 &&
      pl.resident && l->interleave_ranks <= 1 && l->machine_share <= 1 && !pl.pipelined && !pl.brute_walk && !ad)
    pl.which = PTAMD_KERNEL_BVH_PERSISTENT;
  return PTAMD_OK;
}

void lay_out_lds(const ptamd_context* ctx, const DeviceScene& s, bool stats, const AdaptiveParams* ad, LaunchPlan& pl, KParams& p)
{
  if (pl.which != PTAMD_KERNEL_BVH_RESTART) return;
  if (pl.resident) {
    const uint32_t waves = restart_threads(true) / 64u;
    const size_t blocks_wanted = (24u + waves - 1u) / waves;
    const auto fits = [&](size_t scene) { return (((scene + 15u) & ~(size_t)15u) + (size_t)waves * PT_POOL_LDS_BYTES) * blocks_wanted + 1024u <= 160u * 1024u; };
    if ((p.round_form & PT_ROUND_SKIP) && !(ctx->knobs.pool_in_lds && fits(pl.lds + PT_SKIP_ENTRY_BYTES))) p.round_form &= ~(PT_ROUND_SKIP | PT_ROUND_DEFER);
    const size_t scene_lds = pl.lds + ((p.round_form & PT_ROUND_SKIP) ? PT_SKIP_ENTRY_BYTES : 0u);
    if (ad || (ctx->knobs.pool_in_lds && fits(scene_lds))) {
      p.pool_lds_offset = (uint32_t)((scene_lds + 15u) & ~(size_t)15u);
      if (p.pool_lds_offset == 0) p.pool_lds_offset = 16u;
      pl.launch_lds = p.pool_lds_offset + (size_t)waves * PT_POOL_LDS_BYTES;
    }
    return;
  }
  const uint32_t need = choose_wide_nodes(ctx, s, !stats && !pl.fma && !pl.brute_walk && !ctx->d_timeline && !ad, p);
  const uint32_t node_bytes = p.wide8 == 2u ? 64u : 128u;
  const uint32_t waves = restart_threads(false) / 64u;
  const uint32_t share = 160u * 1024u / restart_wide_blocks_per_cu() - 256u;
  const uint32_t pools = (ctx->knobs.pool_in_lds && ctx->knobs.pool_in_lds_wide && !ad) ? waves * PT_POOL_LDS_BYTES : 0u;
  const uint32_t region = kRestartTreeletRegionBytes;
  uint32_t treelet_want = ctx->knobs.treelet_nodes * (128u / node_bytes);
  if (treelet_want > region / node_bytes) treelet_want = region / node_bytes;
  const uint32_t treelet = treelet_want < p.n_nodes4 ? treelet_want : p.n_nodes4;
  const uint32_t treelet_bytes = treelet ? region : 0u;
  uint32_t fit = (share - pools - treelet_bytes) / (waves * 512u);
  if (const char* ev = tuning_env("PTAMD_STACK_LDS")) { int v = std::atoi(ev); if (v >= 1 && (uint32_t)v <= fit) fit = (uint32_t)v; }
  p.treelet_nodes = treelet;
  p.stack_lds_entries = need < fit ? need : fit;
  p.stack_spill_entries = need - p.stack_lds_entries;
  pl.launch_lds = (size_t)treelet_bytes + (size_t)p.stack_lds_entries * waves * 512u;
  if (pools) {
    p.pool_lds_offset = (uint32_t)pl.launch_lds;
    if (!p.pool_lds_offset) p.pool_lds_offset = 16u;
    pl.launch_lds = p.pool_lds_offset + pools;
  }
}

KernelForm form_of(const LaunchPlan& pl, bool stats, bool list, const KParams* p)
{
  return megakernel_form(pl.fma ? (uint32_t)PTAMD_KERNEL_BVH_RESTART_FMA : pl.which, pl.resident, stats, list, pl.launch_lds, p);
}

int blocks_per_cu(ptamd_context* ctx, const LaunchPlan& pl, const KernelForm& form, int& bpc)
{
  ptamd_context::Occupancy& occ = ctx->occupancy[form.cache_slot];
  const size_t key = pl.resident ? pl.launch_lds : (pl.which == PTAMD_KERNEL_BVH_RESTART ? pl.launch_lds + 1u : 0);
  if (occ.blocks_per_cu < 0 || occ.lds != key) {
    int q = -1;
    const hipError_t e = form_blocks_per_cu(form, &q);
    if (e != hipSuccess || q < 1) {
      occ.blocks_per_cu = -1;
      return hip_fail((std::string("occupancy query of the ") + form.name + " kernel").c_str(), e);
    }
    occ.blocks_per_cu = q; occ.lds = key;
  }
  bpc = occ.blocks_per_cu;
  return PTAMD_OK;
}

int size_grid(ptamd_context* ctx, const ptamd_launch* l, const AdaptiveParams* ad, LaunchPlan& pl, KParams& p)
{
  const bool restart = pl.which == PTAMD_KERNEL_BVH_RESTART;
  const uint32_t count = l->frame_count > 1 ? l->frame_count : 1u;
  uint32_t rows = l->row_end - l->row_begin;
  if (l->interleave_ranks > 1u) {
    rows = ptamd_interleaved_rows(l->height, l->interleave_ranks, l->interleave_rank, l->interleave_rows);
    p.ilv_ranks = l->interleave_ranks; p.ilv_rank = l->interleave_rank; p.ilv_rows = l->interleave_rows;
    p.row_begin = 0; p.row_end = rows;
    p.tfb_row0 = l->height - rows;
    p.surf_row0 = 0;
  }
  p.y_limit = l->row_end;
  p.tiles_x = (l->width + PT_TILE_W - 1u) / PT_TILE_W;
  p.n_tiles = p.tiles_x * ((rows + PT_TILE_H - 1u) / PT_TILE_H);
  if (p.n_tiles == 0) return PTAMD_OK;
  if ((uint64_t)p.n_tiles * count >= (1ull << 31)) {
    set_error("ptamd_raytrace: rows x width x frame_count too large for one launch (split the batch)");
    return PTAMD_ERR_LIMIT;
  }
  int bpc = 0;
  const KernelForm form = form_of(pl, false, ad != nullptr, nullptr);
  const int rc = blocks_per_cu(ctx, pl, form, bpc);
  if (rc != PTAMD_OK) return rc;
  pl.waves_per_block = form.ticket_waves;
  uint32_t n_blocks = (uint32_t)ctx->n_cus * (uint32_t)bpc;
  p.sample_count = count;
  p.frame_nb0 = l->frame_nb;
  p.refill_min = ctx->knobs.refill_min ? ctx->knobs.refill_min : (l->bounces >= 5 ? 16u : 64u);
  p.tiles_per_ticket = ad ? 1u : ctx->knobs.tiles_per_ticket;
// ... 28 lines not shown
    PT_HIP(hipStreamSynchronize(pl.stream));
    for (uint32_t k = 0; k < ctx->n_lanes; ++k) PT_HIP(hipStreamSynchronize(ctx->lane[k].get()));
    for (const Stream& is : ctx->internal) if (is) PT_HIP(hipStreamSynchronize(is.get()));
    sc->bytes[i] = 0;
    if (sc->buf[i].alloc(need) != hipSuccess) { (void)hipGetLastError(); return PTAMD_ERR_HIP; }
    sc->bytes[i] = need;
    return PTAMD_OK;
  };
  pl.slab = pl.pipelined ? sc->flip % 3u : 3u;
  if (pl.pipelined) {
    for (int i = 0; i < 3; ++i) {
      PT_HIP(sc->mega_done[i].ensure());
      PT_HIP(sc->resolved[i].ensure());
    }
    bool ok = true;
    for (uint32_t i = 0; i < 3u && ok; ++i) if (need > sc->bytes[i]) ok = grow(i) == PTAMD_OK;
    if (!ok) {
      for (uint32_t i = 0; i < 3u; ++i) { sc->buf[i].reset(); sc->bytes[i] = 0; }
      sc->no_pipeline = true;
      return kReplan;
    }
  } else if (need > sc->bytes[3]) {
    if (pl.capturing) {
      set_error("ptamd_raytrace: a launch cannot size its stream's sample slab inside a graph capture: issue this configuration once eagerly first");
      return PTAMD_ERR_LIMIT;
    }
    if (sc->captured) {
      set_error("ptamd_raytrace: a captured graph pins this stream's sample slab; a larger launch would reallocate it under the graph "
                "(ptamd_release_captured(ctx, stream) once the graph is gone)");
      return PTAMD_ERR_LIMIT;
    }
    if (grow(3u) != PTAMD_OK) return hip_fail("hipMalloc of the sample slab", hipErrorOutOfMemory);
  }
  p.samples_out = sc->buf[pl.slab].get();
  p.pool = reinterpret_cast<float4*>(reinterpret_cast<char*>(p.samples_out) + sample_bytes);
  p.stack_spill = reinterpret_cast<uint2*>(reinterpret_cast<char*>(p.samples_out) + sample_bytes + pool_bytes);
  return PTAMD_OK;
}

int take_slot(ptamd_context* ctx, bool capturing, ptamd_context::SampleScratch* sc, uint32_t& slot)
{
  slot = ctx->ticket_next++ % kTicketRing;
  for (uint32_t tries = 0; ctx->slot_pinned[slot]; ++tries) {
    if (tries >= kTicketRing) { set_error("ptamd_raytrace: every ring slot of ticket heads is pinned by captured graphs (ptamd_release_captured)"); return PTAMD_ERR_LIMIT; }
    slot = ctx->ticket_next++ % kTicketRing;
  }
  if (capturing && sc) { ctx->slot_pinned[slot] = true; sc->pinned_slots.push_back(slot); sc->captured = true; }
  return PTAMD_OK;
}

int issue(ptamd_context* ctx, const DeviceScene& scene, bool stats, const AdaptiveParams* ad, const LaunchPlan& pl, KParams& p)
{
  const bool split = pl.which == PTAMD_KERNEL_BVH_SPLIT, restart = pl.which == PTAMD_KERNEL_BVH_RESTART;
  ptamd_context::SampleScratch* sc = pl.sc;
  int urc = wait_for_update(scene, pl.stream, pl.capturing);
  if (urc != PTAMD_OK) return urc;
  p.round_min = ctx->knobs.round_min;
  p.round_div = ctx->knobs.round_div;
  p.round_defer = ctx->knobs.round_min | ((ctx->knobs.leaf_defer == PT_LEAF_DEFER_AUTO ? 0xFFu : ctx->knobs.leaf_defer) << 8);
  p.round_div_m16 = (65536u + ctx->knobs.round_div - 1u) / ctx->knobs.round_div;
  p.walk_min = ctx->knobs.walk_min;
  p.walk_min4 = ctx->knobs.walk_min4;
  p.tile_counter = ctx->d_tickets.get() + pl.slot;
  if (ad) p.adaptive = ad->block;
  p.n_static = pl.n_blocks * pl.waves_per_block;
  if (split) PT_HIP(hipMemsetD32Async(reinterpret_cast<hipDeviceptr_t>(p.tile_counter), (int)p.n_static, 1, pl.stream));
  hipStream_t mega_stream = pl.stream;
  if (pl.pipelined) {
    mega_stream = pl.stream != nullptr ? ctx->lane[ctx->lane_next++ % ctx->n_lanes].get() : ctx->internal[ctx->lane_next++ & 1u].get();
    sc->flip++;
    if (sc->resolved_valid[pl.slab]) PT_HIP(hipStreamWaitEvent(mega_stream, sc->resolved[pl.slab].get(), 0));
    if ((urc = wait_for_update(scene, mega_stream, false)) != PTAMD_OK) return urc;
  }
  if (!split) {
    p.tile_heads = ctx->d_heads.get() + (size_t)pl.slot * 8u * PT_HEAD_STRIDE;
    if (!ctx->heads_clean[pl.slot]) PT_HIP(hipMemsetD32Async(reinterpret_cast<hipDeviceptr_t>(p.tile_heads), 0, 8u * PT_HEAD_STRIDE, mega_stream));
    ctx->heads_clean[pl.slot] = false;
  }
  if (restart && !pl.fma && ctx->d_timeline && p.n_static <= ctx->timeline_waves) p.timeline = ctx->d_timeline.get();
  if (split) p.tiles_per_ticket = 1;
  const KernelForm form = form_of(pl, stats, ad != nullptr, &p);
  ctx->last_restart_form = form.restart_form < 0 ? -1 : restart_traits(form.restart_form).reports;
  ctx->last_restart_deferred = form.restart_form >= 0 && restart_traits(form.restart_form).defer;
  hipError_t e = launch_form(form, p, pl.n_blocks, restart ? mega_stream : pl.stream);
  if (e == hipSuccess && pl.pipelined) {
    PT_HIP(hipEventRecord(sc->mega_done[pl.slab].get(), mega_stream));
    PT_HIP(hipStreamWaitEvent(pl.stream, sc->mega_done[pl.slab].get(), 0));
  }
  if (e == hipSuccess && (p.sample_count > 1 || restart)) {
    if (ad) {
      AdaptiveParams a = *ad;
      a.samples = p.samples_out;
      a.tile_heads = p.tile_heads;
      e = launch_adaptive_resolve_list(a, pl.stream);
    } else {
      e = launch_resolve(p, pl.stream);
    }
    if (e == hipSuccess && !split) ctx->heads_clean[pl.slot] = true;
    if (e == hipSuccess && pl.pipelined) {
      PT_HIP(hipEventRecord(sc->resolved[pl.slab].get(), pl.stream));
      sc->resolved_valid[pl.slab] = true;
    }
  }
  if (e == hipSuccess && !pl.capturing && ctx->knobs.overlap) {
    PT_HIP(sc->last_done.ensure());
    PT_HIP(hipEventRecord(sc->last_done.get(), pl.stream));
  }
  return e == hipSuccess ? PTAMD_OK : hip_fail("megakernel launch", e);
}

int launch_part(ptamd_context* ctx, const ptamd_launch* l, bool stats, bool later_chunk, const AdaptiveParams* ad, const LaunchPlan& resolved)
{
  LaunchPlan pl = resolved;
  KParams p;
  int rc;
  if (persistent_family(pl.which)) {
    do {
      pl = resolved;
      fill_launch(ctx, l, stats, pl, p);
      if ((rc = plan_stream(ctx, l, stats, later_chunk, ad, pl)) != PTAMD_OK) return rc;
      lay_out_lds(ctx, ctx->scenes[l->scene_id], stats, ad, pl, p);
      if ((rc = size_grid(ctx, l, ad, pl, p)) != PTAMD_OK || p.n_tiles == 0) return rc;
      rc = bind_slab(ctx, l, pl, p);
    } while (rc == kReplan);
    if (rc != PTAMD_OK || (rc = take_slot(ctx, pl.capturing, pl.sc, pl.slot)) != PTAMD_OK) return rc;
    return issue(ctx, ctx->scenes[l->scene_id], stats, ad, pl, p);
  }
  fill_launch(ctx, l, stats, pl, p);
  if (ctx->scenes[l->scene_id].updated_valid &&
      (rc = wait_for_update(ctx->scenes[l->scene_id], pl.stream, stream_is_capturing(pl.stream))) != PTAMD_OK) return rc;
  const KernelForm form = form_of(pl, stats, false, &p);
  uint32_t n_blocks = 0;
  if (pl.which == PTAMD_KERNEL_BVH_BLOCKWISE) {
    const uint32_t rows = l->row_end - l->row_begin;
    const uint32_t st_rows = (form.threads / 64u) * 2u;
    p.tiles_x = (l->width + 31u) / 32u;
    p.n_tiles = p.tiles_x * ((rows + st_rows - 1u) / st_rows);
    if (p.n_tiles == 0) return PTAMD_OK;
    int bpc = 0;
    if ((rc = blocks_per_cu(ctx, pl, form, bpc)) != PTAMD_OK || (rc = take_slot(ctx, false, nullptr, pl.slot)) != PTAMD_OK) return rc;
    n_blocks = std::min((uint32_t)ctx->n_cus * (uint32_t)bpc, p.n_tiles);
    p.tile_counter = ctx->d_tickets.get() + pl.slot;
    PT_HIP(hipMemsetD32Async(reinterpret_cast<hipDeviceptr_t>(p.tile_counter), (int)n_blocks, 1, pl.stream));
  }
  const hipError_t e = launch_form(form, p, n_blocks, pl.stream);
  return e == hipSuccess ? PTAMD_OK : hip_fail("megakernel launch", e);
}

}

int do_launch(ptamd_context* ctx, const ptamd_launch* l, bool stats, const AdaptiveParams* ad)
{
  int rc = validate_launch(ctx, l);
  LaunchPlan resolved;
  if (rc != PTAMD_OK || (rc = settle_margins(ctx->scenes[l->scene_id], static_cast<hipStream_t>(l->stream), "ptamd_raytrace")) != PTAMD_OK ||
      (rc = resolve_kernel(ctx, l, stats, ad, resolved)) != PTAMD_OK) return rc;
  PT_HIP(hipSetDevice(ctx->device));
  const uint32_t part_frames = persistent_family(resolved.which) ? kMaxFramesPerSlab : 1u;
  for (uint32_t k0 = 0; k0 == 0 || k0 < l->frame_count; k0 += part_frames) {
    ptamd_launch part = *l;
    part.frame_nb = l->frame_nb + k0;
    part.frame_count = std::min(l->frame_count - k0, part_frames);
    if (k0 > 0) part.reset_accumulation = 0;
    if ((rc = launch_part(ctx, &part, stats, k0 > 0, ad, resolved)) != PTAMD_OK) return rc;
  }
  return PTAMD_OK;
// ... 146 lines not shown
```

### cuda-pathtracer_amd/csrc/ptamd_scene.cpp

```cpp
#include "ptamd_host.h"
#include "pt_refit.h"
#include "pt_refit_device.h"

#include <cmath>
#include <cstring>

namespace ptamd {

bool far_origin_camera(const DeviceScene& s, const ptamd_camera& cam)
{
  const float cam_far = std::fmax(std::fabs(cam.position.x), std::fmax(std::fabs(cam.position.y), std::fabs(cam.position.z))) +
                        std::fabs(cam.aperture);
  return !(margins_cover(s.extent, s.margin_floor, cam_far) && margins_cover(s.extent, s.margin_floor, s.reach)) && s.n_faces != 0;
}

int settle_margins(DeviceScene& s, hipStream_t stream, const char* who)
{
  if (!s.margins_pending) return PTAMD_OK;
  if (stream_is_capturing(stream)) {
    set_error(std::string(who) + ": the scene's margins are pending behind ptamd_scene_update_device and a capture cannot wait for "
              "them: render the scene once, or call ptamd_scene_quality, outside the capture");
    return PTAMD_ERR_LIMIT;
  }
  PT_HIP(hipEventSynchronize(s.margin_ready[s.margin_slot].get()));
// ... 611 lines not shown
  const void* src[6] = { t.bvh.nodes.data(), t.bvh.tris.data(), t.bvh.nodes4.data(), t.brute.data(), t.shade.data(), scalars };
  const uint64_t size[6] = { t.bvh.nodes.size() * 4u, t.bvh.tris.size() * 4u, t.bvh.nodes4.size() * 4u, t.brute.size() * 4u, t.shade.size() * 4u, 16u };
  const uint64_t room = *bytes;
  *bytes = size[which];
  if (!out) return PTAMD_OK;
  if (room < size[which]) { set_error("ptamd_host_scene_refit: the buffer is smaller than the table"); return PTAMD_ERR_ARG; }
  if (size[which]) std::memcpy(out, src[which], size[which]);
  return PTAMD_OK;
}

int ptamd_upload_cubemap(ptamd_context* ctx, const float* faces, uint32_t size, uint32_t* out_cubemap_id)
{
  if (!ctx || !faces || !out_cubemap_id || size == 0 || size > 16384) { set_error("ptamd_upload_cubemap: bad argument"); return PTAMD_ERR_ARG; }
  PT_HIP(hipSetDevice(ctx->device));
  DeviceCubemap c;
  c.size = size;
  if (size == 1) {
    c.uniform = true;
    for (int f = 1; f < 6; ++f) c.uniform = c.uniform && std::memcmp(faces + f * 4, faces, 12) == 0;
    std::memcpy(c.color, faces, 12);
  }
  int rc = upload(c.faces, faces, (size_t)6 * size * size * 16);
  if (rc != PTAMD_OK) return rc;
  ctx->cubemaps.push_back(std::move(c));
  *out_cubemap_id = (uint32_t)ctx->cubemaps.size() - 1;
  return PTAMD_OK;
}

int ptamd_scene_info_get(ptamd_context* ctx, uint32_t scene_id, ptamd_scene_info* out)
{
  if (!ctx || !out || !live_scene(ctx, scene_id)) { set_error("ptamd_scene_info_get: bad argument"); return PTAMD_ERR_ARG; }
  *out = ctx->scenes[scene_id].info;
  return PTAMD_OK;
}

int ptamd_scene_desc_is_flat(const ptamd_scene_desc* sc, int32_t* out_flat)
{
  if (!sc || !out_flat || (sc->n_faces && !sc->faces) || (sc->n_materials && !sc->materials) || (sc->n_textures && !sc->textures)) {
    set_error("ptamd_scene_desc_is_flat: null argument or table");
    return PTAMD_ERR_ARG;
  }
  for (uint32_t i = 0; i < sc->n_faces; ++i) {
    const uint32_t m = sc->faces[i].material_id;
    if (m >= sc->n_materials || sc->materials[m].diffuse_spec_map < 0 || (uint32_t)sc->materials[m].diffuse_spec_map >= sc->n_textures) {
      set_error("ptamd_scene_desc_is_flat: material or texture id out of range");
      return PTAMD_ERR_ARG;
    }
  }
  *out_flat = scene_is_flat(sc) ? 1 : 0;
  return PTAMD_OK;
}

int ptamd_scene_is_flat(ptamd_context* ctx, uint32_t scene_id, uint32_t cubemap_id, int32_t* out_flat)
{
  if (!ctx || !out_flat || !live_scene(ctx, scene_id) || cubemap_id >= ctx->cubemaps.size()) {
    set_error("ptamd_scene_is_flat: bad argument");
    return PTAMD_ERR_ARG;
  }
  *out_flat = ctx->knobs.flat_round && ctx->scenes[scene_id].flat && ctx->cubemaps[cubemap_id].uniform ? 1 : 0;
  return PTAMD_OK;
}

int ptamd_scene_skip_count(ptamd_context* ctx, uint32_t scene_id, uint32_t* out)
{
  if (!ctx || !out || !live_scene(ctx, scene_id)) { set_error("ptamd_scene_skip_count: bad argument"); return PTAMD_ERR_ARG; }
  *out = ctx->scenes[scene_id].n_skipped;
  return PTAMD_OK;
}

int ptamd_last_restart_form(ptamd_context* ctx, int32_t* out)
{
  if (!ctx || !out) { set_error("ptamd_last_restart_form: null argument"); return PTAMD_ERR_ARG; }
  *out = ctx->last_restart_form;
  return PTAMD_OK;
}

int ptamd_last_restart_deferred(ptamd_context* ctx, int32_t* out)
{
  if (!ctx || !out) { set_error("ptamd_last_restart_deferred: null argument"); return PTAMD_ERR_ARG; }
  *out = ctx->last_restart_deferred ? 1 : 0;
  return PTAMD_OK;
}

int ptamd_scene_cull_count(ptamd_context* ctx, uint32_t scene_id, uint32_t* out)
{
  if (!ctx || !out || !live_scene(ctx, scene_id)) { set_error("ptamd_scene_cull_count: bad argument"); return PTAMD_ERR_ARG; }
  *out = ctx->scenes[scene_id].n_culled;
  return PTAMD_OK;
}

}
```

### cuda-pathtracer_amd/csrc/ptamd_tuning.cpp

```cpp
#include "ptamd_tuning.h"
#include "../host/ptamd_internal.h"

#include <cstdlib>
#include <cstring>

namespace ptamd {

const char* tuning_env(const char* name)
{
  const char* gate = std::getenv("PTAMD_TUNING");
  if (!gate || std::atoi(gate) != 1) return nullptr;
  return std::getenv(name);
}

namespace {

enum KnobKind {
  kSwitch,
  kClamped,
  kKernel,
  kSkipWord,
  kOpenUnit,
};

struct Knob {
  const char* name;
  KnobKind kind;
  bool TuningSettings::* flag;
  uint32_t TuningSettings::* number;
  float TuningSettings::* real;
  int lo, hi;
};

constexpr Knob on_off(const char* name, bool TuningSettings::* f) { return { name, kSwitch, f, nullptr, nullptr, 0, 1 }; }
constexpr Knob number(const char* name, KnobKind kind, uint32_t TuningSettings::* f, int lo, int hi) { return { name, kind, nullptr, f, nullptr, lo, hi }; }

using S = TuningSettings;
constexpr Knob kKnobs[] = {
  on_off("PTAMD_GAMMA_TABLE", &S::gamma_table),
  on_off("PTAMD_OVERLAP", &S::overlap),
  number("PTAMD_REFILL_MIN", kClamped, &S::refill_min, 1, 64),
  number("PTAMD_DEFAULT_KERNEL", kKernel, &S::default_kernel, 1, 6),
  number("PTAMD_ROUND_MIN", kClamped, &S::round_min, 1, 64),
  number("PTAMD_ROUND_DIV", kClamped, &S::round_div, 1, 64),
  number("PTAMD_WALK_MIN", kClamped, &S::walk_min, 1, 64),
  number("PTAMD_WALK_MIN4", kClamped, &S::walk_min4, 1, 64),
  number("PTAMD_LEAF_DEFER", kClamped, &S::leaf_defer, 0, 64),
  on_off("PTAMD_SHORT_RCP", &S::short_rcp),
  on_off("PTAMD_WIDE8", &S::wide8),
  on_off("PTAMD_WIDE4Q", &S::wide4q),
  on_off("PTAMD_RS_GENERIC", &S::generic_round),
  on_off("PTAMD_RS_FLAT", &S::flat_round),
  number("PTAMD_SKIP", kSkipWord, &S::skip_mode, 0, 0),
  { "PTAMD_SKIP_THRESHOLD", kOpenUnit, nullptr, nullptr, &S::skip_threshold, 0, 1 },
  on_off("PTAMD_POOL_LDS", &S::pool_in_lds),
  on_off("PTAMD_POOL_LDS_WIDE", &S::pool_in_lds_wide),
  number("PTAMD_TREELET", kClamped, &S::treelet_nodes, 0, 1024),
  number("PTAMD_XCD_REGIONS", kClamped, &S::xcd_regions, 0, 2),
  number("PTAMD_TILES_PER_TICKET", kClamped, &S::tiles_per_ticket, 1, 1024),
};

}

void read_tuning_knobs(TuningSettings& s)
{
  s = TuningSettings();
  for (const Knob& k : kKnobs) {
    const char* e = tuning_env(k.name);
    if (!e) continue;
    const int v = std::atoi(e);
    switch (k.kind) {
      case kSwitch: s.*k.flag = v != 0; break;
      case kClamped: s.*k.number = (uint32_t)(v < k.lo ? k.lo : (v > k.hi ? k.hi : v)); break;
      case kKernel:
        if (v >= k.lo && v <= k.hi) { s.*k.number = (uint32_t)v; s.default_kernel_is_builtin = false; }
        break;
      case kSkipWord:
        s.*k.number = !std::strcmp(e, "root") ? PTAMD_SKIP_ROOT : (!std::strcmp(e, "all") ? PTAMD_SKIP_ALL : (!std::strcmp(e, "0") ? PTAMD_SKIP_SET : PTAMD_SKIP_DEFAULT));
        break;
      case kOpenUnit: {
        const float f = (float)std::atof(e);
        if (f > (float)k.lo && f < (float)k.hi) s.*k.real = f;
        break;
      }
    }
  }
}

}
```

### cuda-pathtracer_amd/csrc/ptamd_tuning.h

```cpp
#pragma once

#include "ptamd.h"

namespace ptamd {

struct TuningSettings {
  bool gamma_table = true;
  bool overlap = true;
  uint32_t refill_min = 0;
  uint32_t default_kernel = PTAMD_KERNEL_BVH_RESTART;
  bool default_kernel_is_builtin = true;
  uint32_t round_min = 16, round_div = 4;
  uint32_t walk_min = 7;
  uint32_t leaf_defer = 0xFFFFFFFFu;
  uint32_t walk_min4 = 16;
  bool short_rcp = true;
  bool wide8 = false;
  bool wide4q = false;
  bool generic_round = false;
  bool flat_round = true;
  uint32_t skip_mode = PTAMD_SKIP_DEFAULT;
  float skip_threshold = 0.0f;
  bool pool_in_lds = true;
  bool pool_in_lds_wide = false;
  uint32_t treelet_nodes = 512;
  uint32_t xcd_regions = 0;
  uint32_t tiles_per_ticket = 1;
};

void read_tuning_knobs(TuningSettings& s);

}
```

### cuda-pathtracer_amd/native.py

```python
from __future__ import annotations

import ctypes as C
import os
import sys

_HERE = os.path.dirname(os.path.abspath(__file__))
LIB_PATH = os.path.join(_HERE, "libptamd.so")


class PtamdError(RuntimeError):

    def __init__(self, status: int, message: str):
        super().__init__(f"ptamd status {status}: {message}")
        self.status = status


PTAMD_OK, PTAMD_ERR_ARG, PTAMD_ERR_HIP, PTAMD_ERR_IO, PTAMD_ERR_LIMIT = 0, 1, 2, 3, 4
KERNEL_AUTO, KERNEL_BRUTE_FORCE, KERNEL_BVH, KERNEL_BVH_PERSISTENT, KERNEL_BVH_BLOCKWISE, KERNEL_BVH_SPLIT, KERNEL_BVH_RESTART = 0, 1, 2, 3, 4, 5, 6
KERNEL_BVH_RESTART_FMA = 7


class Float3(C.Structure):
    _fields_ = [("x", C.c_float), ("y", C.c_float), ("z", C.c_float)]

# ... 198 lines not shown
    "ptamd_scene_rig_morph": (C.c_int, [C.c_void_p, C.POINTER(SceneRigMorphDesc)]),
    "ptamd_host_morph_faces": (C.c_int, [C.POINTER(Face), C.c_uint32, C.POINTER(MorphTarget), C.c_uint32, C.POINTER(C.c_float),
                                         C.POINTER(Face)]),
    "ptamd_scene_update_lights": (C.c_int, [C.c_void_p, C.POINTER(SceneLightsDesc)]),
    "ptamd_scene_quality": (C.c_int, [C.c_void_p, C.c_uint32, C.c_void_p, C.POINTER(SceneQualityInfo)]),
    "ptamd_host_scene_quality": (C.c_int, [C.POINTER(SceneDesc), C.POINTER(Face), C.POINTER(C.c_double)]),
    "ptamd_scene_margins": (C.c_int, [C.c_void_p, C.c_uint32, C.POINTER(C.c_float)]),
    "ptamd_scene_release": (C.c_int, [C.c_void_p, C.c_uint32]),
    "ptamd_scene_table_read": (C.c_int, [C.c_void_p, C.c_uint32, C.c_uint32, C.c_void_p, C.POINTER(C.c_uint64)]),
    "ptamd_host_scene_refit": (C.c_int, [C.POINTER(SceneDesc), C.POINTER(Face), C.POINTER(Face), C.c_uint32, C.c_void_p,
                                         C.POINTER(C.c_uint64)]),
    "ptamd_host_bvh_refit_trace": (C.c_int, [C.POINTER(Face), C.POINTER(Face), C.c_uint32, C.POINTER(C.c_float), C.c_uint32,
                                             C.POINTER(C.c_int32), C.POINTER(C.c_int32)]),
    "ptamd_upload_cubemap": (C.c_int, [C.c_void_p, C.POINTER(C.c_float), C.c_uint32, C.POINTER(C.c_uint32)]),
    "ptamd_setup_function_tables": (C.c_int, [C.c_void_p]),
    "ptamd_raytrace": (C.c_int, [C.c_void_p, C.c_void_p, C.c_uint32, C.c_uint32, C.POINTER(Camera), C.c_uint32,
                                 C.c_uint32, C.c_void_p, C.c_void_p, C.c_int32, C.c_uint32]),
    "ptamd_raytrace_ex": (C.c_int, [C.c_void_p, C.POINTER(Launch)]),
    "ptamd_reset_frame_counter": (C.c_int, [C.c_void_p]),
    "ptamd_wang_hash": (C.c_uint32, [C.c_uint32]),
    "ptamd_interleaved_rows": (C.c_uint32, [C.c_uint32, C.c_uint32, C.c_uint32, C.c_uint32]),
    "ptamd_release_captured": (C.c_int, [C.c_void_p, C.c_void_p]),
    "ptamd_raytrace_stats": (C.c_int, [C.c_void_p, C.POINTER(Launch), C.POINTER(TraceStats)]),
    "ptamd_scene_info_get": (C.c_int, [C.c_void_p, C.c_uint32, C.POINTER(SceneInfo)]),
    "ptamd_scene_desc_is_flat": (C.c_int, [C.POINTER(SceneDesc), C.POINTER(C.c_int32)]),
    "ptamd_scene_is_flat": (C.c_int, [C.c_void_p, C.c_uint32, C.c_uint32, C.POINTER(C.c_int32)]),
    "ptamd_set_timeline": (C.c_int, [C.c_void_p, C.c_uint32]),
    "ptamd_read_timeline": (C.c_int, [C.c_void_p, C.POINTER(C.c_uint64), C.c_uint32, C.POINTER(C.c_uint32)]),
    "ptamd_device_error_count": (C.c_int, [C.c_void_p, C.POINTER(C.c_uint64)]),
    "ptamd_phase_cycles": (C.c_int, [C.c_void_p, C.POINTER(C.c_uint64)]),
    "ptamd_gamma_table_selftest": (C.c_int, [C.c_void_p, C.POINTER(C.c_uint64), C.POINTER(C.c_uint64)]),
    "ptamd_trace_rays": (C.c_int, [C.c_void_p, C.c_uint32, C.c_uint32, C.POINTER(C.c_float), C.c_uint32,
                                   C.POINTER(C.c_int32)]),
    "ptamd_host_bvh_trace": (C.c_int, [C.POINTER(Face), C.c_uint32, C.POINTER(C.c_float), C.c_uint32,
                                       C.POINTER(C.c_int32), C.POINTER(C.c_uint64)]),
    "ptamd_host_bvh4_trace": (C.c_int, [C.POINTER(Face), C.c_uint32, C.POINTER(C.c_float), C.c_uint32,
                                       C.POINTER(C.c_int32), C.POINTER(C.c_uint64)]),
    "ptamd_host_bvh4q_trace": (C.c_int, [C.POINTER(Face), C.c_uint32, C.POINTER(C.c_float), C.c_uint32,
                                       C.POINTER(C.c_int32), C.POINTER(C.c_uint64)]),
    "ptamd_host_bvh8_trace": (C.c_int, [C.POINTER(Face), C.c_uint32, C.POINTER(C.c_float), C.c_uint32,
                                       C.POINTER(C.c_int32), C.POINTER(C.c_uint64)]),
    "ptamd_host_origin_reach": (C.c_int, [C.POINTER(Face), C.c_uint32, C.POINTER(Light), C.c_uint32, C.POINTER(C.c_float)]),
    "ptamd_trace_rays_queue": (C.c_int, [C.c_void_p, C.c_uint32, C.c_void_p, C.c_uint32, C.c_void_p, C.c_uint32, C.c_uint32, C.c_void_p,
                                        C.POINTER(C.c_uint32)]),
    "ptamd_denoise": (C.c_int, [C.c_void_p, C.POINTER(DenoiseDesc)]),
    "ptamd_render_features": (C.c_int, [C.c_void_p, C.c_uint32, C.c_uint32, C.POINTER(Camera), C.c_uint32, C.c_uint32,
                                        C.c_void_p, C.c_void_p, C.c_void_p]),
    "ptamd_host_denoise": (C.c_int, [C.c_void_p, C.c_void_p, C.POINTER(DenoiseDesc), C.c_void_p, C.c_void_p]),
    "ptamd_get_frame_counter": (C.c_int, [C.c_void_p, C.POINTER(C.c_uint32)]),
    "ptamd_denoise_history_create": (C.c_int, [C.c_void_p, C.c_uint32, C.c_uint32, C.POINTER(C.c_void_p)]),
    "ptamd_denoise_history_destroy": (C.c_int, [C.c_void_p, C.c_void_p]),
    "ptamd_denoise_history_reset": (C.c_int, [C.c_void_p, C.c_void_p, C.c_void_p]),
    "ptamd_denoise_history_view_of": (C.c_int, [C.c_void_p, C.POINTER(DenoiseHistoryView)]),
    "ptamd_denoise_temporal": (C.c_int, [C.c_void_p, C.POINTER(DenoiseTemporalDesc)]),
    "ptamd_host_denoise_temporal": (C.c_int, [C.c_void_p, C.c_void_p, C.POINTER(DenoiseTemporalDesc), C.POINTER(DenoiseHistoryView),
                                              C.c_void_p, C.c_void_p]),
    "ptamd_denoise_temporal_motion": (C.c_int, [C.c_void_p, C.POINTER(DenoiseTemporalDesc)]),
    "ptamd_denoise_history_geometry_read": (C.c_int, [C.c_void_p, C.c_void_p, C.POINTER(C.c_uint64), C.POINTER(C.c_uint32),
                                                      C.POINTER(C.c_uint64)]),
    "ptamd_host_denoise_temporal_motion": (C.c_int, [C.c_void_p, C.c_void_p, C.POINTER(DenoiseTemporalDesc), C.POINTER(DenoiseHistoryView),
                                                     C.c_void_p, C.c_void_p, C.c_uint32, C.c_void_p, C.c_void_p]),
    "ptamd_adaptive_create": (C.c_int, [C.c_void_p, C.c_uint32, C.c_uint32, C.POINTER(C.c_void_p)]),
    "ptamd_adaptive_destroy": (C.c_int, [C.c_void_p, C.c_void_p]),
    "ptamd_adaptive_reset": (C.c_int, [C.c_void_p, C.c_void_p, C.c_void_p]),
    "ptamd_adaptive_view_of": (C.c_int, [C.c_void_p, C.POINTER(AdaptiveView)]),
    "ptamd_render_adaptive": (C.c_int, [C.c_void_p, C.POINTER(AdaptiveDesc)]),
    "ptamd_adaptive_select": (C.c_int, [C.c_void_p, C.POINTER(AdaptiveDesc)]),
    "ptamd_adaptive_resolve": (C.c_int, [C.c_void_p, C.POINTER(AdaptiveDesc), C.c_void_p]),
    "ptamd_host_adaptive_select": (C.c_int, [C.POINTER(AdaptiveDesc), C.c_void_p, C.c_void_p, C.c_void_p, C.c_void_p]),
    "ptamd_device_alloc": (C.c_int, [C.c_void_p, C.c_size_t, C.POINTER(C.c_void_p)]),
    "ptamd_device_free": (C.c_int, [C.c_void_p, C.c_void_p]),
    "ptamd_device_memset": (C.c_int, [C.c_void_p, C.c_void_p, C.c_int, C.c_size_t, C.c_void_p]),
    "ptamd_device_to_host": (C.c_int, [C.c_void_p, C.c_void_p, C.c_void_p, C.c_size_t, C.c_void_p]),
    "ptamd_host_to_device": (C.c_int, [C.c_void_p, C.c_void_p, C.c_void_p, C.c_size_t, C.c_void_p]),
    "ptamd_stream_synchronize": (C.c_int, [C.c_void_p, C.c_void_p]),
    "ptamd_scene_skip_count": (C.c_int, [C.c_void_p, C.c_uint32, C.POINTER(C.c_uint32)]),
    "ptamd_host_skip_trace": (C.c_int, [C.POINTER(Face), C.POINTER(Face), C.c_uint32, C.c_uint32, C.c_float, C.c_void_p,
                                        C.POINTER(C.c_float), C.c_uint32, C.POINTER(C.c_int32), C.POINTER(C.c_uint64),
                                        C.POINTER(C.c_uint32), C.c_void_p, C.c_void_p]),
    "ptamd_scene_cull_count": (C.c_int, [C.c_void_p, C.c_uint32, C.POINTER(C.c_uint32)]),
    "ptamd_last_restart_form": (C.c_int, [C.c_void_p, C.POINTER(C.c_int32)]),
    "ptamd_host_faces_away": (C.c_int, [C.c_void_p, C.c_uint32, C.c_void_p]),
    "ptamd_last_restart_deferred": (C.c_int, [C.c_void_p, C.POINTER(C.c_int32)]),
    "ptamd_host_skip_events": (C.c_int, [C.POINTER(Face), C.c_uint32, C.c_uint32, C.c_float, C.POINTER(C.c_float), C.c_uint32,
                                         C.c_void_p, C.c_void_p, C.POINTER(C.c_uint64)]),
    "ptamd_host_round_threshold": (C.c_uint32, [C.c_uint32, C.c_uint32, C.c_uint32]),
    "ptamd_host_round_leaf_defer": (C.c_uint32, [C.c_uint32, C.c_uint32]),
    "ptamd_host_round_leaf_phase_runs": (C.c_int, [C.c_int, C.c_uint32, C.c_uint32]),
    "ptamd_host_round_ends": (C.c_int, [C.c_uint32, C.c_uint32]),
    "ptamd_host_round_pending_pack": (C.c_uint32, [C.c_uint32, C.c_uint32]),
    "ptamd_host_round_pending_unpack": (C.c_int, [C.c_uint32, C.POINTER(C.c_uint32), C.POINTER(C.c_uint32)]),
}

_lib = None


def load() -> C.CDLL:
    global _lib
    if _lib is not None:
        return _lib
    if "torch" not in sys.modules and os.environ.get("PTAMD_NO_TORCH_PRELOAD") != "1":
        try:
            import torch
        except Exception:
            pass
    if not os.path.exists(LIB_PATH):
        raise ImportError(
            f"{LIB_PATH} is missing: the HIP library has not been built. "
            "Run `python -c \"import __graft_entry__ as g; g.build()\"` (or `make lib`). "
            "There is no CPU fallback for the render path.")
    lib = C.CDLL(LIB_PATH)
    for name, (res, args) in SIGNATURES.items():
        fn = getattr(lib, name)
        fn.restype = res
        fn.argtypes = args
    _lib = lib
    return lib


def check(status: int) -> None:
    if status != PTAMD_OK:
        raise PtamdError(status, load().ptamd_get_last_error().decode("utf-8", "replace"))
```

### cuda-pathtracer_amd/render.py

```python
from __future__ import annotations

import ctypes as C
from typing import Optional

import numpy as np

from . import native as N
from .scene import FACE_DTYPE, LIGHT_DTYPE, HostScene

POST_NONE, POST_GRAYSCALE, POST_SEPIA, POST_INVERT = 0, 1, 2, 3
REFERENCE_BOUNCES = 3


def _ptr(buf) -> int:
    if isinstance(buf, int):
        return buf
    if hasattr(buf, "data_ptr"):
        if not buf.is_cuda:
            raise ValueError("output buffers must live in device memory (no CPU path exists)")
        if not buf.is_contiguous():
            raise ValueError("output buffers must be contiguous")
        return buf.data_ptr()
    raise TypeError(f"unsupported buffer type {type(buf)!r}")

# ... 54 lines not shown
            raise ValueError("update_scene_device takes a tensor in device memory (CPU tensors: update_scene)")
        if faces.device.index != self.device:
            raise ValueError(f"the faces live on {faces.device}, the context on device {self.device}")
        if not ((faces.dtype == torch.float32 and faces.dim() == 2 and faces.shape[1] == 28) or
                (faces.dtype == torch.uint8 and faces.dim() == 2 and faces.shape[1] == 112)):
            raise ValueError("faces must be float32 of shape (n, 28) or uint8 of shape (n, 112)")
        if not faces.is_contiguous():
            raise ValueError("faces must be contiguous")
        d = N.SceneUpdateDeviceDesc()
        d.scene_id = scene_id
        d.faces = faces.data_ptr(); d.n_faces = faces.shape[0]
        d.stream = _stream_handle(stream)
        N.check(self._lib.ptamd_scene_update_device(self._h, C.byref(d)))

    def scene_rig(self, scene_id: int, host_scene, group_sizes=None) -> "SceneRig":
        return SceneRig(self, scene_id, host_scene, group_sizes)

    def update_lights(self, scene_id: int, lights, stream=None) -> None:
        lights = np.ascontiguousarray(lights.lights if isinstance(lights, HostScene) else lights, dtype=LIGHT_DTYPE)
        d = N.SceneLightsDesc()
        d.scene_id = scene_id
        d.lights = lights.ctypes.data_as(C.POINTER(N.Light)); d.n_lights = len(lights)
        d.stream = _stream_handle(stream)
        N.check(self._lib.ptamd_scene_update_lights(self._h, C.byref(d)))

    def scene_quality(self, scene_id: int, stream=None):
        q = N.SceneQualityInfo()
        N.check(self._lib.ptamd_scene_quality(self._h, scene_id, _stream_handle(stream), C.byref(q)))
        return q.built, q.now

    def scene_margins(self, scene_id: int) -> np.ndarray:
        out = (C.c_float * 4)()
        N.check(self._lib.ptamd_scene_margins(self._h, scene_id, out))
        return np.array(out[:], dtype=np.float32)

    def release_scene(self, scene_id: int) -> None:
        N.check(self._lib.ptamd_scene_release(self._h, scene_id))

    def read_scene_tables(self, scene_id: int) -> dict:
        out = {}
        for which, name in enumerate(N.TABLE_NAMES):
            n = C.c_uint64(0)
            N.check(self._lib.ptamd_scene_table_read(self._h, scene_id, which, None, C.byref(n)))
            buf = np.zeros(n.value, np.uint8)
            N.check(self._lib.ptamd_scene_table_read(self._h, scene_id, which, buf.ctypes.data, C.byref(n)))
            out[name] = buf
        return out

    def upload_cubemap(self, faces: np.ndarray) -> int:
        faces = np.ascontiguousarray(faces, dtype=np.float32)
        if faces.ndim != 4 or faces.shape[0] != 6 or faces.shape[1] != faces.shape[2] or faces.shape[3] != 4:
            raise ValueError("cubemap must be float32[6, size, size, 4]")
        cid = C.c_uint32()
        N.check(self._lib.ptamd_upload_cubemap(self._h, faces.ctypes.data_as(C.POINTER(C.c_float)),
                                               faces.shape[1], C.byref(cid)))
        return cid.value

    def setup_function_tables(self) -> None:
        N.check(self._lib.ptamd_setup_function_tables(self._h))

    def scene_info(self, scene_id: int) -> dict:
        info = N.SceneInfo()
        N.check(self._lib.ptamd_scene_info_get(self._h, scene_id, C.byref(info)))
        return {n: getattr(info, n) for n, _ in N.SceneInfo._fields_}

    def scene_skip_count(self, scene_id: int) -> int:
        out = C.c_uint32(0)
        N.check(self._lib.ptamd_scene_skip_count(self._h, scene_id, C.byref(out)))
        return out.value

    def scene_cull_count(self, scene_id: int) -> int:
        out = C.c_uint32(0)
        N.check(self._lib.ptamd_scene_cull_count(self._h, scene_id, C.byref(out)))
        return out.value

    def last_restart_form(self) -> int:
        out = C.c_int32(-1)
        N.check(self._lib.ptamd_last_restart_form(self._h, C.byref(out)))
        return out.value

    def last_restart_deferred(self) -> bool:
        out = C.c_int32(0)
        N.check(self._lib.ptamd_last_restart_deferred(self._h, C.byref(out)))
        return out.value != 0

    def scene_is_flat(self, scene_id: int, cubemap_id: int) -> bool:
        out = C.c_int32()
        N.check(self._lib.ptamd_scene_is_flat(self._h, scene_id, cubemap_id, C.byref(out)))
        return out.value != 0

    def raytrace(self, array, scene_id: int, cubemap_id: int, cam: N.Camera, width: int, height: int,
                 stream, temporal_framebuffer, moved: bool, post_id: int) -> None:
        N.check(self._lib.ptamd_raytrace(self._h, _ptr(array), scene_id, cubemap_id, C.byref(cam), width, height,
                                         _stream_handle(stream), _ptr(temporal_framebuffer),
                                         1 if moved else 0, post_id))

    def reset_frame_counter(self) -> None:
        N.check(self._lib.ptamd_reset_frame_counter(self._h))

    def make_launch(self, array, temporal_framebuffer, scene_id: int, cubemap_id: int, cam: N.Camera,
                    width: int, height: int, frame_nb: int, bounces: int = REFERENCE_BOUNCES,
                    moved: bool = False, post_id: int = POST_NONE, stream=None,
                    rows: Optional[tuple] = None, kernel: int = N.KERNEL_AUTO,
                    band_local_buffers: bool = False, frame_count: int = 1, machine_share: int = 0,
                    interleave: Optional[tuple] = None, reset_accumulation: bool = False, no_pipelining: bool = False) -> N.Launch:
        l = N.Launch()
        l.surface_rgba8 = _ptr(array)
        l.temporal_framebuffer = _ptr(temporal_framebuffer)
        l.stream = _stream_handle(stream)
        l.camera = cam
        l.scene_id, l.cubemap_id = scene_id, cubemap_id
        l.width, l.height = width, height
        l.row_begin, l.row_end = rows if rows is not None else (0, height)
        l.frame_nb, l.bounces = frame_nb, bounces
        l.moved, l.post_id, l.kernel = (1 if moved else 0), post_id, kernel
        l.band_local_buffers = 1 if band_local_buffers else 0
        l.frame_count = frame_count
        l.machine_share = machine_share
        if interleave is not None:
            l.interleave_ranks, l.interleave_rank, l.interleave_rows = interleave
        l.reset_accumulation = 1 if reset_accumulation else 0
        l.no_pipelining = 1 if no_pipelining else 0
        return l

    def raytrace_ex(self, launch: N.Launch) -> None:
        N.check(self._lib.ptamd_raytrace_ex(self._h, C.byref(launch)))

    def frame_counter(self) -> int:
        out = C.c_uint32()
        N.check(self._lib.ptamd_get_frame_counter(self._h, C.byref(out)))
        return out.value

    def denoise(self, surface, temporal_framebuffer, scene_id: int, cubemap_id: int, cam: N.Camera, width: int, height: int,
                frame_nb: int, levels: int = 5, post_id: int = POST_NONE, sigma_n: float = 0.0, sigma_l: float = 0.0,
                sigma_x: float = 0.0, linear=None, stream=None) -> None:
        d = N.DenoiseDesc()
        d.temporal_framebuffer = _ptr(temporal_framebuffer)
        d.frame_nb = frame_nb
        d.camera = cam
        d.scene_id, d.cubemap_id, d.width, d.height = scene_id, cubemap_id, width, height
        d.surface_rgba8 = _ptr(surface)
        d.linear_rgb = _ptr(linear) if linear is not None else None
        d.stream = _stream_handle(stream)
        d.post_id, d.levels = post_id, levels
        d.sigma_n, d.sigma_l, d.sigma_x = sigma_n, sigma_l, sigma_x
        N.check(self._lib.ptamd_denoise(self._h, C.byref(d)))

    def adaptive_state(self, width: int, height: int) -> "AdaptiveState":
        return AdaptiveState(self, width, height)

    def denoise_history(self, width: int, height: int) -> "DenoiseHistory":
        return DenoiseHistory(self, width, height)

    def denoise_temporal(self, surface, temporal_framebuffer, scene_id: int, cubemap_id: int, cam: N.Camera, width: int,
                         height: int, frame_nb: int, history: "DenoiseHistory", levels: int = 5, post_id: int = POST_NONE,
                         sigma_n: float = 0.0, sigma_l: float = 0.0, sigma_x: float = 0.0, alpha_color: float = 0.0,
                         alpha_moments: float = 0.0, reset_history: bool = False, history_length=None, linear=None,
                         stream=None, motion: bool = False) -> None:
        if history.ctx is not self:
            raise ValueError("the history belongs to another context")
        d = N.DenoiseTemporalDesc()
        b = d.base
        b.temporal_framebuffer = _ptr(temporal_framebuffer)
        b.frame_nb = frame_nb
        b.camera = cam
        b.scene_id, b.cubemap_id, b.width, b.height = scene_id, cubemap_id, width, height
# ... 797 lines not shown
```

### include/ptamd.h

```cpp
#ifndef PTAMD_H
#define PTAMD_H

#include <stddef.h>
#include <stdint.h>

#ifdef __cplusplus
extern "C" {
#endif

typedef enum {
  PTAMD_OK = 0,
  PTAMD_ERR_ARG = 1,
  PTAMD_ERR_HIP = 2,
  PTAMD_ERR_IO = 3,
  PTAMD_ERR_LIMIT = 4
} ptamd_status;


typedef struct { float x, y, z; } ptamd_float3;
typedef struct { float x, y; } ptamd_float2;

typedef struct {
  ptamd_float3 vertices[3];
  ptamd_float3 normals[3];
// ... 337 lines not shown
  float* moments;
  float* normal;
  float* position;
} ptamd_denoise_history_view;

int ptamd_denoise_history_view_of(const ptamd_denoise_history* history, ptamd_denoise_history_view* out);

int ptamd_host_denoise_temporal(const float* features, const float* temporal_framebuffer, const ptamd_denoise_temporal_desc* desc,
                                ptamd_denoise_history_view* history, float* linear_rgb, uint8_t* rgba8);

int ptamd_denoise_temporal_motion(ptamd_context* ctx, const ptamd_denoise_temporal_desc* desc);

int ptamd_denoise_history_geometry_read(ptamd_denoise_history* history, void* out, uint64_t* bytes, uint32_t* scene_id, uint64_t* serial);

int ptamd_host_denoise_temporal_motion(const float* features, const float* temporal_framebuffer, const ptamd_denoise_temporal_desc* desc,
                                       ptamd_denoise_history_view* history, const float* tris_now, const float* tris_prev, uint32_t n_faces,
                                       float* linear_rgb, uint8_t* rgba8);

typedef struct ptamd_adaptive_state ptamd_adaptive_state;

int ptamd_adaptive_create(ptamd_context* ctx, uint32_t width, uint32_t height, ptamd_adaptive_state** out);
int ptamd_adaptive_destroy(ptamd_context* ctx, ptamd_adaptive_state* state);
int ptamd_adaptive_reset(ptamd_context* ctx, ptamd_adaptive_state* state, void* stream);

typedef struct {
  uint32_t width, height;
  uint32_t* counts;
  float* moments;
  uint32_t* list;
  uint32_t* active_count;
} ptamd_adaptive_view;

int ptamd_adaptive_view_of(const ptamd_adaptive_state* state, ptamd_adaptive_view* out);

typedef struct {
  void* surface_rgba8;
  float* temporal_framebuffer;
  void* stream;
  ptamd_camera camera;
  uint32_t scene_id, cubemap_id;
  uint32_t width, height;
  uint32_t bounces;
  uint32_t post_id;
  uint32_t kernel;
  ptamd_adaptive_state* state;
  uint32_t min_spp, max_spp;
  uint32_t samples_per_round;
  uint32_t rounds;
  float threshold;
  float err_floor;
  uint32_t dilate;
  uint32_t* active_counts;
} ptamd_adaptive_desc;

int ptamd_render_adaptive(ptamd_context* ctx, const ptamd_adaptive_desc* desc);

int ptamd_adaptive_select(ptamd_context* ctx, const ptamd_adaptive_desc* desc);

int ptamd_adaptive_resolve(ptamd_context* ctx, const ptamd_adaptive_desc* desc, float* linear_rgb);

int ptamd_host_adaptive_select(const ptamd_adaptive_desc* desc, const uint32_t* counts, const float* moments, uint32_t* list,
                               uint32_t* active_count);

int ptamd_get_frame_counter(ptamd_context* ctx, uint32_t* out);

int ptamd_device_alloc(ptamd_context* ctx, size_t bytes, void** out);
int ptamd_device_free(ptamd_context* ctx, void* p);
int ptamd_device_memset(ptamd_context* ctx, void* p, int value, size_t bytes, void* stream);
int ptamd_device_to_host(ptamd_context* ctx, void* dst_host, const void* src_dev, size_t bytes, void* stream);
int ptamd_host_to_device(ptamd_context* ctx, void* dst_dev, const void* src_host, size_t bytes, void* stream);
int ptamd_stream_synchronize(ptamd_context* ctx, void* stream);

#define PTAMD_SKIP_SET 0u
#define PTAMD_SKIP_DEFAULT 1u
#define PTAMD_SKIP_ROOT 2u
#define PTAMD_SKIP_ALL 3u
#define PTAMD_SKIP_CULLED 0x100u
#define PTAMD_FORM_FLAT_SKIP 9
#define PTAMD_FORM_PLAIN_SKIP 10
int ptamd_scene_skip_count(ptamd_context* ctx, uint32_t scene_id, uint32_t* out);
int ptamd_scene_cull_count(ptamd_context* ctx, uint32_t scene_id, uint32_t* out);
int ptamd_last_restart_form(ptamd_context* ctx, int32_t* out);
int ptamd_last_restart_deferred(ptamd_context* ctx, int32_t* out);
int ptamd_host_skip_trace(const ptamd_face* faces, const ptamd_face* faces_refit, uint32_t n_faces, uint32_t mode, float threshold,
                          const uint8_t* skip_in, const float* rays, uint32_t n, int32_t* out, uint64_t* counters,
                          uint32_t* n_nodes, uint8_t* skip_out, uint32_t* words_out);
int ptamd_host_faces_away(const float* edges, uint32_t n, uint8_t* out);

int ptamd_host_skip_events(const ptamd_face* faces, uint32_t n_faces, uint32_t mode, float threshold, const float* rays, uint32_t n,
                           uint32_t* offsets, uint32_t* events, uint64_t* n_events);
uint32_t ptamd_host_round_threshold(uint32_t n_start, uint32_t round_min, uint32_t round_div);
uint32_t ptamd_host_round_leaf_defer(uint32_t knob, uint32_t t_eff);
int ptamd_host_round_leaf_phase_runs(int first, uint32_t unfinished, uint32_t leaf_defer);
int ptamd_host_round_ends(uint32_t unfinished, uint32_t t_eff);
uint32_t ptamd_host_round_pending_pack(uint32_t leaf_code, uint32_t continuation);
int ptamd_host_round_pending_unpack(uint32_t node, uint32_t* leaf_code, uint32_t* continuation);

#ifdef __cplusplus
}
#endif
#endif
```

Baseline: 14620.

## Add tight specialised traversal round for flat deferring skip form in separate unit

Adds a new restart form (FLAT_SKIP_TIGHT) with a dedicated traversal round. It keeps LDS byte-address states instead of node indices, stages per-octant entry states as LDS offsets, always uses the asm leaf test, and drops the stats and generic branches. The form is compiled in a separate translation unit so the lean kernel gets its own register allocation, and it is on by default when small_det and the flat/skip/defer flags are all set. Exchange: more code paths and a second build unit, plus a risk of changed scheduling or register pressure.

Measured after the change: 15030 (median of 6 runs). 1.03x the previous value.

```diff
diff --git a/cuda-pathtracer_amd/csrc/pt_device.h b/cuda-pathtracer_amd/csrc/pt_device.h
--- a/cuda-pathtracer_amd/csrc/pt_device.h
+++ b/cuda-pathtracer_amd/csrc/pt_device.h
@@ -392,6 +392,12 @@
 #define PT_ROUND_FLAT 2u
 #define PT_ROUND_SKIP 4u
 #define PT_ROUND_DEFER 8u
+#define PT_ROUND_TIGHT 16u
+inline bool round_form_tight(uint32_t round_form, uint32_t small_det, bool knob)
+{
+  const uint32_t needs = PT_ROUND_FLAT | PT_ROUND_SKIP | PT_ROUND_DEFER;
+  return knob && small_det != 0u && (round_form & needs) == needs;
+}
 #define PT_SKIP_ENTRY_BYTES 32u
 
 #define PT_RS_PLAIN 0
@@ -408,7 +414,8 @@
 #define PT_RS_FLAT_SKIP_DEFER 11
 #define PT_RS_PLAIN_SKIP_DEFER 12
 #define PT_RS_STATS_DEFER 13
-#define PT_RS_FORMS 14
+#define PT_RS_FLAT_SKIP_TIGHT 14
+#define PT_RS_FORMS 15
 
 struct RestartTraits {
   bool stats;
@@ -420,24 +427,26 @@
   bool flat;
   bool skip;
   bool defer;
+  bool tight;
   int reports;
   bool resident, streamed, contracted;
 };
 constexpr RestartTraits kRestartForms[] = {
-  { false, false, false, 0, false, true,  false, false, false, PT_RS_PLAIN,      true,  true,  true },
-  { true,  false, false, 0, false, false, false, false, false, PT_RS_STATS,      true,  true,  false },
-  { false, true,  false, 0, false, false, false, false, false, PT_RS_STAMPS,     true,  true,  false },
-  { false, false, true,  0, false, false, false, false, false, PT_RS_BRUTE,      true,  true,  true },
-  { false, false, false, 1, false, false, false, false, false, PT_RS_WIDE8,      false, true,  false },
-  { false, false, false, 2, false, false, false, false, false, PT_RS_WIDE4Q,     false, true,  false },
-  { false, false, false, 0, false, false, false, false, false, PT_RS_GENERIC,    true,  false, true },
-  { false, false, false, 0, true,  false, false, false, false, PT_RS_LIST,       true,  true,  false },
-  { false, false, false, 0, false, true,  true,  false, false, PT_RS_FLAT,       true,  false, false },
-  { false, false, false, 0, false, true,  true,  true,  false, PT_RS_FLAT_SKIP,  true,  false, false },
-  { false, false, false, 0, false, true,  false, true,  false, PT_RS_PLAIN_SKIP, true,  false, false },
-  { false, false, false, 0, false, true,  true,  true,  true,  PT_RS_FLAT_SKIP,  true,  false, false },
-  { false, false, false, 0, false, true,  false, true,  true,  PT_RS_PLAIN_SKIP, true,  false, false },
-  { true,  false, false, 0, false, false, false, false, true,  PT_RS_STATS,      true,  false, false },
+  { false, false, false, 0, false, true,  false, false, false, false, PT_RS_PLAIN,      true,  true,  true },
+  { true,  false, false, 0, false, false, false, false, false, false, PT_RS_STATS,      true,  true,  false },
+  { false, true,  false, 0, false, false, false, false, false, false, PT_RS_STAMPS,     true,  true,  false },
+  { false, false, true,  0, false, false, false, false, false, false, PT_RS_BRUTE,      true,  true,  true },
+  { false, false, false, 1, false, false, false, false, false, false, PT_RS_WIDE8,      false, true,  false },
+  { false, false, false, 2, false, false, false, false, false, false, PT_RS_WIDE4Q,     false, true,  false },
+  { false, false, false, 0, false, false, false, false, false, false, PT_RS_GENERIC,    true,  false, true },
+  { false, false, false, 0, true,  false, false, false, false, false, PT_RS_LIST,       true,  true,  false },
+  { false, false, false, 0, false, true,  true,  false, false, false, PT_RS_FLAT,       true,  false, false },
+  { false, false, false, 0, false, true,  true,  true,  false, false, PT_RS_FLAT_SKIP,  true,  false, false },
+  { false, false, false, 0, false, true,  false, true,  false, false, PT_RS_PLAIN_SKIP, true,  false, false },
+  { false, false, false, 0, false, true,  true,  true,  true,  false, PT_RS_FLAT_SKIP,  true,  false, false },
+  { false, false, false, 0, false, true,  false, true,  true,  false, PT_RS_PLAIN_SKIP, true,  false, false },
+  { true,  false, false, 0, false, false, false, false, true,  false, PT_RS_STATS,      true,  false, false },
+  { false, false, false, 0, false, true,  true,  true,  true,  true,  PT_RS_FLAT_SKIP,  true,  false, false },
 };
 static_assert(sizeof kRestartForms / sizeof kRestartForms[0] == PT_RS_FORMS, "one row per PT_RS_* number");
 constexpr RestartTraits restart_traits(int variant) { return kRestartForms[variant]; }
@@ -460,6 +469,7 @@
   if (!lds_resident && p && p->wide8) return { full(p->wide8 == 2u ? PT_RS_WIDE4Q : PT_RS_WIDE8), false };
   if (!lds_resident) return { PT_RS_PLAIN, false };
   if (p && !restart_shipped_launch(*p)) return { PT_RS_GENERIC, true };
+  if (defers && (p->round_form & PT_ROUND_FLAT) && (p->round_form & PT_ROUND_TIGHT)) return { PT_RS_FLAT_SKIP_TIGHT, true };
   if (defers) return { (p->round_form & PT_ROUND_FLAT) ? PT_RS_FLAT_SKIP_DEFER : PT_RS_PLAIN_SKIP_DEFER, true };
   if (p && (p->round_form & PT_ROUND_SKIP) && !contracted) return { (p->round_form & PT_ROUND_FLAT) ? PT_RS_FLAT_SKIP : PT_RS_PLAIN_SKIP, true };
   if (p && (p->round_form & PT_ROUND_FLAT)) return { full(PT_RS_FLAT), true };
diff --git a/cuda-pathtracer_amd/csrc/pt_kernels.hip b/cuda-pathtracer_amd/csrc/pt_kernels.hip
--- a/cuda-pathtracer_amd/csrc/pt_kernels.hip
+++ b/cuda-pathtracer_amd/csrc/pt_kernels.hip
@@ -4,7 +4,11 @@
 
 #include <utility>
 
-#ifndef PT_FMA_BUILD
+#if defined(PT_FMA_BUILD) || defined(PT_TIGHT_BUILD)
+#define PT_SIDE_UNIT 1
+#endif
+
+#ifndef PT_SIDE_UNIT
 #include "pt_denoise.h"
 #endif
 
@@ -331,17 +335,22 @@
   w.node = walk_lds_node(lds_nodes, state);
 }
 
+PT_DEV void walk_leaf_asm(const float4* tris, Walk& w, uint32_t leaf_first, uint32_t leaf_count, uint32_t stride = 3u )
+{
+  for (uint32_t k = 0; k < leaf_count; ++k) {
+    const float4* r = tris + (leaf_first + k) * stride;
+    const float4 a = r[0], b = r[1];
+    const float2 c = *reinterpret_cast<const float2*>(r + 2);
+    mt_test_asm(a, b, c, w.o, w.d, w.best);
+  }
+}
+
 template <bool STATS, bool ASM = false>
 PT_DEV void walk_leaf(const float4* tris, Walk& w, uint32_t leaf_first, uint32_t leaf_count, uint32_t& n_tris,
                       uint32_t& wave_tri_iters, bool small_det = false, uint32_t stride = 3u )
 {
   if (ASM && !STATS && PT_ASM_LEAF && small_det) {
-    for (uint32_t k = 0; k < leaf_count; ++k) {
-      const float4* r = tris + (leaf_first + k) * stride;
-      const float4 a = r[0], b = r[1];
-      const float2 c = *reinterpret_cast<const float2*>(r + 2);
-      mt_test_asm(a, b, c, w.o, w.d, w.best);
-    }
+    walk_leaf_asm(tris, w, leaf_first, leaf_count, stride);
     return;
   }
   for (uint32_t k = 0; k < leaf_count; ++k) {
@@ -805,7 +814,7 @@
   }
 }
 
-template <int KIND, bool LDS_RESIDENT, bool COMPACT = false, bool SKIP = false>
+template <int KIND, bool LDS_RESIDENT, bool COMPACT = false, bool SKIP = false, bool ENTRY_STATES = false>
 PT_DEV void stage_scene(const KParams& p, float4* s_mem_, const float4*& s_nodes, const float4*& s_tris)
 {
   float4* const s_mem = SKIP ? s_mem_ + PT_SKIP_ENTRY_BYTES / 16u : s_mem_;
@@ -820,7 +829,8 @@
         const uint32_t* relinked = reinterpret_cast<const uint32_t*>(p.nodes + p.n_nodes * 4);
         if (SKIP && threadIdx.x < 8u) {
           const uint32_t e = relinked[p.n_nodes * 8u + threadIdx.x];
-          reinterpret_cast<uint32_t*>(s_mem_)[threadIdx.x] = e == 0xFFFFu ? PT_END : e;
+          if (ENTRY_STATES) reinterpret_cast<uint32_t*>(s_mem_)[threadIdx.x] = e == 0xFFFFu ? 0xFFFFu : base + e * 32u;
+          else reinterpret_cast<uint32_t*>(s_mem_)[threadIdx.x] = e == 0xFFFFu ? PT_END : e;
         }
         if (base + p.n_nodes * 32u > 0x8000u || p.n_bvh_tris > 2047u) __builtin_trap();
         for (uint32_t i = threadIdx.x; i < p.n_nodes; i += blockDim.x) {
@@ -1074,6 +1084,36 @@
   best = w.best;
   node = w.node;
   if (STATS) { cnt.idle3[0] += w.idle_unstarted; cnt.idle3[1] += w.idle_finished; cnt.idle3[2] += w.idle_parked; }
+}
+
+#define PT_WALK_FRESH 0xFFFFFFFFu
+PT_DEV void traverse_round_tight(const float4* nodes, const float4* tris, const uint32_t* entries, uint32_t n_nodes, f3 o, f3 d, Best& best, uint32_t& pos,
+                                 uint32_t round_min, uint32_t leaf_defer_knob, uint32_t round_div, uint32_t round_div_m16, uint32_t walk_min)
+{
+  Walk w;
+  walk_init(w, o, d, n_nodes, true);
+  asm volatile("" : "+v"(w.oct));
+  w.best = best;
+  const uint32_t entry = entries[w.oct];
+  if (pos == PT_WALK_FRESH) pos = entry;
+  const uint32_t n_start = (uint32_t)__popcll(__ballot(pos != 0xFFFFu));
+  const uint32_t t_eff = round_threshold(n_start, round_min, round_div, round_div_m16);
+  const uint32_t leaf_defer = round_leaf_defer(leaf_defer_knob, t_eff);
+  const bool pending = round_is_pending(pos);
+  uint32_t state = pending ? round_pending_leaf(pos) : pos;
+  const uint32_t lnk = walk_lds_link_offset(w);
+  uint32_t leaf_first, leaf_count;
+  for (bool first = true;; first = false) {
+    walk_to_leaf_lds_state(state, lnk, w, leaf_first, leaf_count, walk_min);
+    if (first && pending) state = round_pending_continuation(pos);
+    const unsigned long long walking = __builtin_amdgcn_ballot_w64(state != 0xFFFFu), parked = __builtin_amdgcn_ballot_w64(leaf_count != 0u);
+    if (!round_leaf_phase_runs(first, (uint32_t)__popcll(walking | parked), leaf_defer)) break;
+    if (leaf_count != 0u) walk_leaf_asm(tris, w, leaf_first, leaf_count);
+    leaf_count = 0u;
+    if (round_ends((uint32_t)__popcll(walking), t_eff)) break;
+  }
+  pos = leaf_count != 0u ? round_pending_pack(0x8000u | (leaf_count << 11) | leaf_first, state) : state;
+  best = w.best;
 }
 
 template <bool STATS, bool NODES_IN_LDS, bool DEFER = false>
@@ -1649,6 +1689,9 @@
   constexpr bool STATS = FORM.stats;
   constexpr uint32_t THREADS = LDS_RESIDENT ? PT_RS_THREADS : PT_RS4_THREADS;
   constexpr bool DEFER = LDS_RESIDENT && FORM.defer;
+  constexpr bool TIGHT = DEFER && FORM.tight;
+  static_assert(!FORM.tight || (FORM.defer && FORM.skip && FORM.lean && !FORM.stats && PT_ASM_LEAF), "the tight round is the flat deferring skip form's");
+  constexpr uint32_t WALK_OVER = TIGHT ? 0xFFFFu : PT_END;
   constexpr bool SKIP = LDS_RESIDENT && FORM.skip;
   constexpr bool FLAT = LDS_RESIDENT && FORM.flat;
   constexpr bool LEAN = LDS_RESIDENT && FORM.lean;
@@ -1658,7 +1701,7 @@
   const float4* s_nodes;
   const float4* s_tris;
   PT_STAMP(0);
-  stage_scene<2, LDS_RESIDENT, LDS_RESIDENT && !STATS, SKIP>(p, s_mem, s_nodes, s_tris);
+  stage_scene<2, LDS_RESIDENT, LDS_RESIDENT && !STATS, SKIP, TIGHT>(p, s_mem, s_nodes, s_tris);
   constexpr bool WIDE = !LDS_RESIDENT;
 
   const uint32_t lane = threadIdx.x & 63u;
@@ -1691,7 +1734,7 @@
   bool walking = false;
   Best best;
   best.t = PT_MAX_DIST; best.u = best.v = 0.f; best.idx = PT_END;
-  uint32_t node = PT_END;
+  uint32_t node = WALK_OVER;
   uint32_t pool_rd = 64u, tile_x0 = 0, tile_y0 = 0, tile_k = 0;
   uint32_t tile_row_delta = 0;
   uint32_t tile = 0, tile_end = 0;
@@ -1827,7 +1870,8 @@
     if (!idle) {
       if (!walking) {
         best.t = PT_MAX_DIST; best.u = 0.f; best.v = 0.f; best.idx = PT_END;
-        if (SKIP) node = reinterpret_cast<const uint32_t*>(s_mem)[(st.d.x < 0.f ? 1u : 0u) | (st.d.y < 0.f ? 2u : 0u) | (st.d.z < 0.f ? 4u : 0u)];
+        if (TIGHT) node = PT_WALK_FRESH;
+        else if (SKIP) node = reinterpret_cast<const uint32_t*>(s_mem)[(st.d.x < 0.f ? 1u : 0u) | (st.d.y < 0.f ? 2u : 0u) | (st.d.z < 0.f ? 4u : 0u)];
         else node = p.n_nodes ? 0u : PT_END;
         cur = p.n_nodes4 ? 0u : PT_NONE;
         sp = 0u;
@@ -1841,14 +1885,17 @@
       } else if (WIDE) {
         traverse_round4<STATS, FORM.wide>(p, p.nodes4, s_tris, stk, st.o, st.d, best, cur, sp, p.round_min, p.round_div, p.round_div_m16, p.walk_min4, p.small_det != 0u, cnt);
         node = cur == PT_NONE ? PT_END : 0u;
+      } else if constexpr (TIGHT) {
+        traverse_round_tight(s_nodes, s_tris, reinterpret_cast<const uint32_t*>(s_mem), p.n_nodes, st.o, st.d, best, node, p.round_min, (p.round_defer >> 8) == 0xFFu ? PT_LEAF_DEFER_AUTO : p.round_defer >> 8,
+                             p.round_div, p.round_div_m16, p.walk_min);
       } else {
         traverse_round<STATS, LDS_RESIDENT, DEFER>(s_nodes, s_tris, p.n_nodes, st.o, st.d, best, node, DEFER ? p.round_defer : p.round_min, p.round_div, p.round_div_m16, p.walk_min, p.small_det != 0u, cnt);
       }
       if (STATS) {
         if (lane == (uint32_t)(__ffsll((long long)__ballot(1)) - 1)) cnt.fetch_events++;
-        if (node == PT_END) cnt.fetch_rays++;
-      }
-      if (node == PT_END) {
+        if (node == WALK_OVER) cnt.fetch_rays++;
+      }
+      if (node == WALK_OVER) {
         long long tl0 = 0;
         if (STATS) tl0 = clock64();
         const float r1 = path_pre<FIXED>(p, st);
@@ -2371,7 +2418,7 @@
   out[i] = make_int4(kind, index, (int)f_as_u(nr.t), 0);
 }
 
-#ifndef PT_FMA_BUILD
+#ifndef PT_SIDE_UNIT
 
 template <int KIND>
 __global__ void __launch_bounds__(256) pt_features_kernel(PT_KERNEL_PARAMS, float4* feat, float* rays)
@@ -2436,7 +2483,7 @@
 
 
 #define PT_FN(...) reinterpret_cast<const void*>(__VA_ARGS__)
-#ifndef PT_FMA_BUILD
+#ifndef PT_SIDE_UNIT
 static const void* const kTileEntries[2][2][2] = {
   { { PT_FN(pt_megakernel<1, false, false, PT_TILE_THREADS>), PT_FN(pt_megakernel<1, false, true, PT_TILE_THREADS>) },
     { PT_FN(pt_megakernel<1, true, false, PT_TILE_THREADS>), PT_FN(pt_megakernel<1, true, true, PT_TILE_THREADS>) } },
@@ -2451,16 +2498,25 @@
 static const void* const kBlockwiseEntries[2][2] = {
   { PT_FN(pt_megakernel_blockwise<false, false>), PT_FN(pt_megakernel_blockwise<false, true>) },
   { PT_FN(pt_megakernel_blockwise<true, false>), PT_FN(pt_megakernel_blockwise<true, true>) } };
+#endif
+#ifdef PT_FMA_BUILD
+constexpr bool kContracted = true;
+#else
 constexpr bool kContracted = false;
+#endif
+#ifdef PT_TIGHT_BUILD
+constexpr bool kTightUnit = true;
 #else
-constexpr bool kContracted = true;
+constexpr bool kTightUnit = false;
 #endif
 
 template <int V>
 static const void* restart_entry_of(bool lds_resident)
 {
   constexpr RestartTraits FORM = restart_traits(V);
-  if constexpr (FORM.contracted || !kContracted) {
+  if constexpr (FORM.tight && !kTightUnit) {
+    if constexpr (!kContracted) return ptamd_tight_restart_entry(V, lds_resident ? 1 : 0);
+  } else if constexpr ((FORM.contracted || !kContracted) && FORM.tight == kTightUnit) {
     if constexpr (FORM.resident) { if (lds_resident) return PT_FN(pt_megakernel_restart<true, V>); }
     if constexpr (FORM.streamed) { if (!lds_resident) return PT_FN(pt_megakernel_restart<false, V>); }
   }
@@ -2481,7 +2537,7 @@
 uint32_t restart_threads(bool lds_resident) { return lds_resident ? PT_RS_THREADS : PT_RS4_THREADS; }
 uint32_t restart_wide_blocks_per_cu() { return (PT_RS4_WAVES_PER_EU * 256u) / PT_RS4_THREADS; }
 
-static KernelForm restart_form(bool lds_resident, bool stats, bool list, size_t lds_bytes, const KParams* p)
+[[maybe_unused]] static KernelForm restart_form(bool lds_resident, bool stats, bool list, size_t lds_bytes, const KParams* p)
 {
   const RestartForm launched = restart_select(lds_resident, stats, list, kContracted, p);
   const RestartForm queried = restart_select(lds_resident, false, list, kContracted, nullptr);
@@ -2493,7 +2549,7 @@
   return f;
 }
 
-#ifndef PT_FMA_BUILD
+#ifndef PT_SIDE_UNIT
 KernelForm megakernel_form(uint32_t kernel, bool lds_resident, bool stats, bool list, size_t lds_bytes, const KParams* p)
 {
   const int r = lds_resident ? 1 : 0, s = stats ? 1 : 0;
@@ -2645,11 +2701,18 @@
   return hipGetLastError();
 }
 
+#elif defined(PT_FMA_BUILD)
+}
+extern "C" void ptamd_fma_restart_form(int lds_resident, size_t lds_bytes, const ptamd_fma::KParams* p, ptamd_fma::KernelForm* out)
+{
+  *out = ptamd::restart_form(lds_resident != 0, false, false, lds_bytes, p);
+}
+namespace ptamd {
 #else
 }
-extern "C" void ptamd_fma_restart_form(int lds_resident, size_t lds_bytes, const ptamd_fma::KParams* p, ptamd_fma::KernelForm* out)
-{
-  *out = ptamd::restart_form(lds_resident != 0, false, false, lds_bytes, p);
+extern "C" const void* ptamd_tight_restart_entry(int variant, int lds_resident)
+{
+  return ptamd::restart_entry(variant, lds_resident != 0);
 }
 namespace ptamd {
 #endif
diff --git a/cuda-pathtracer_amd/csrc/pt_kernels_tight.hip b/cuda-pathtracer_amd/csrc/pt_kernels_tight.hip
--- /dev/null
+++ b/cuda-pathtracer_amd/csrc/pt_kernels_tight.hip
@@ -0,0 +1,3 @@
+#define PT_TIGHT_BUILD 1
+#define ptamd ptamd_tight
+#include "pt_kernels.hip"
diff --git a/cuda-pathtracer_amd/csrc/pt_launch.h b/cuda-pathtracer_amd/csrc/pt_launch.h
--- a/cuda-pathtracer_amd/csrc/pt_launch.h
+++ b/cuda-pathtracer_amd/csrc/pt_launch.h
@@ -50,3 +50,4 @@
 }
 
 extern "C" void ptamd_fma_restart_form(int lds_resident, size_t lds_bytes, const ptamd::KParams* p, ptamd::KernelForm* out);
+extern "C" const void* ptamd_tight_restart_entry(int variant, int lds_resident);
diff --git a/cuda-pathtracer_amd/csrc/ptamd_host.h b/cuda-pathtracer_amd/csrc/ptamd_host.h
--- a/cuda-pathtracer_amd/csrc/ptamd_host.h
+++ b/cuda-pathtracer_amd/csrc/ptamd_host.h
@@ -92,6 +92,7 @@
   std::vector<ptamd::DeviceCubemap> cubemaps;
   uint32_t frame_counter = 0;
   bool last_restart_deferred = false;
+  bool last_restart_tight = false;
   int32_t last_restart_form = -1;
   ptamd::DeviceBuffer<unsigned long long> d_stats;
   ptamd::DeviceBuffer<float> d_gamma;
diff --git a/cuda-pathtracer_amd/csrc/ptamd_launch.cpp b/cuda-pathtracer_amd/csrc/ptamd_launch.cpp
--- a/cuda-pathtracer_amd/csrc/ptamd_launch.cpp
+++ b/cuda-pathtracer_amd/csrc/ptamd_launch.cpp
@@ -196,6 +196,7 @@
   p.round_form = (ctx->knobs.generic_round ? PT_ROUND_GENERIC : 0u) | (ctx->knobs.flat_round && s.flat && ctx->cubemaps[l->cubemap_id].uniform ? PT_ROUND_FLAT : 0u);
   const bool defer = ctx->knobs.leaf_defer != 0u && (ctx->knobs.leaf_defer != PT_LEAF_DEFER_AUTO || (p.round_form & PT_ROUND_FLAT));
   if (s.links && pl.resident) p.round_form |= PT_ROUND_SKIP | (defer ? PT_ROUND_DEFER : 0u);
+  if (round_form_tight(p.round_form, p.small_det, ctx->knobs.tight_round)) p.round_form |= PT_ROUND_TIGHT;
 }
 
 int plan_stream(ptamd_context* ctx, const ptamd_launch* l, bool stats, bool later_chunk, const AdaptiveParams* ad, LaunchPlan& pl)
@@ -240,7 +241,7 @@
     const uint32_t waves = restart_threads(true) / 64u;
     const size_t blocks_wanted = (24u + waves - 1u) / waves;
     const auto fits = [&](size_t scene) { return (((scene + 15u) & ~(size_t)15u) + (size_t)waves * PT_POOL_LDS_BYTES) * blocks_wanted + 1024u <= 160u * 1024u; };
-    if ((p.round_form & PT_ROUND_SKIP) && !(ctx->knobs.pool_in_lds && fits(pl.lds + PT_SKIP_ENTRY_BYTES))) p.round_form &= ~(PT_ROUND_SKIP | PT_ROUND_DEFER);
+    if ((p.round_form & PT_ROUND_SKIP) && !(ctx->knobs.pool_in_lds && fits(pl.lds + PT_SKIP_ENTRY_BYTES))) p.round_form &= ~(PT_ROUND_SKIP | PT_ROUND_DEFER | PT_ROUND_TIGHT);
     const size_t scene_lds = pl.lds + ((p.round_form & PT_ROUND_SKIP) ? PT_SKIP_ENTRY_BYTES : 0u);
     if (ad || (ctx->knobs.pool_in_lds && fits(scene_lds))) {
       p.pool_lds_offset = (uint32_t)((scene_lds + 15u) & ~(size_t)15u);
@@ -435,6 +436,7 @@
   const KernelForm form = form_of(pl, stats, ad != nullptr, &p);
   ctx->last_restart_form = form.restart_form < 0 ? -1 : restart_traits(form.restart_form).reports;
   ctx->last_restart_deferred = form.restart_form >= 0 && restart_traits(form.restart_form).defer;
+  ctx->last_restart_tight = form.restart_form >= 0 && restart_traits(form.restart_form).tight;
   hipError_t e = launch_form(form, p, pl.n_blocks, restart ? mega_stream : pl.stream);
   if (e == hipSuccess && pl.pipelined) {
     PT_HIP(hipEventRecord(sc->mega_done[pl.slab].get(), mega_stream));
diff --git a/cuda-pathtracer_amd/csrc/ptamd_scene.cpp b/cuda-pathtracer_amd/csrc/ptamd_scene.cpp
--- a/cuda-pathtracer_amd/csrc/ptamd_scene.cpp
+++ b/cuda-pathtracer_amd/csrc/ptamd_scene.cpp
@@ -717,6 +717,13 @@
   return PTAMD_OK;
 }
 
+int ptamd_last_restart_tight(ptamd_context* ctx, int32_t* out)
+{
+  if (!ctx || !out) { set_error("ptamd_last_restart_tight: null argument"); return PTAMD_ERR_ARG; }
+  *out = ctx->last_restart_tight ? 1 : 0;
+  return PTAMD_OK;
+}
+
 int ptamd_scene_cull_count(ptamd_context* ctx, uint32_t scene_id, uint32_t* out)
 {
   if (!ctx || !out || !live_scene(ctx, scene_id)) { set_error("ptamd_scene_cull_count: bad argument"); return PTAMD_ERR_ARG; }
diff --git a/cuda-pathtracer_amd/csrc/ptamd_tuning.cpp b/cuda-pathtracer_amd/csrc/ptamd_tuning.cpp
--- a/cuda-pathtracer_amd/csrc/ptamd_tuning.cpp
+++ b/cuda-pathtracer_amd/csrc/ptamd_tuning.cpp
@@ -51,6 +51,7 @@
   on_off("PTAMD_WIDE4Q", &S::wide4q),
   on_off("PTAMD_RS_GENERIC", &S::generic_round),
   on_off("PTAMD_RS_FLAT", &S::flat_round),
+  on_off("PTAMD_RS_TIGHT", &S::tight_round),
   number("PTAMD_SKIP", kSkipWord, &S::skip_mode, 0, 0),
   { "PTAMD_SKIP_THRESHOLD", kOpenUnit, nullptr, nullptr, &S::skip_threshold, 0, 1 },
   on_off("PTAMD_POOL_LDS", &S::pool_in_lds),
diff --git a/cuda-pathtracer_amd/csrc/ptamd_tuning.h b/cuda-pathtracer_amd/csrc/ptamd_tuning.h
--- a/cuda-pathtracer_amd/csrc/ptamd_tuning.h
+++ b/cuda-pathtracer_amd/csrc/ptamd_tuning.h
@@ -18,6 +18,7 @@
   bool wide8 = false;
   bool wide4q = false;
   bool generic_round = false;
+  bool tight_round = true;
   bool flat_round = true;
   uint32_t skip_mode = PTAMD_SKIP_DEFAULT;
   float skip_threshold = 0.0f;
diff --git a/cuda-pathtracer_amd/native.py b/cuda-pathtracer_amd/native.py
--- a/cuda-pathtracer_amd/native.py
+++ b/cuda-pathtracer_amd/native.py
@@ -304,6 +304,7 @@
     "ptamd_last_restart_form": (C.c_int, [C.c_void_p, C.POINTER(C.c_int32)]),
     "ptamd_host_faces_away": (C.c_int, [C.c_void_p, C.c_uint32, C.c_void_p]),
     "ptamd_last_restart_deferred": (C.c_int, [C.c_void_p, C.POINTER(C.c_int32)]),
+    "ptamd_last_restart_tight": (C.c_int, [C.c_void_p, C.POINTER(C.c_int32)]),
     "ptamd_host_skip_events": (C.c_int, [C.POINTER(Face), C.c_uint32, C.c_uint32, C.c_float, C.POINTER(C.c_float), C.c_uint32,
                                          C.c_void_p, C.c_void_p, C.POINTER(C.c_uint64)]),
     "ptamd_host_round_threshold": (C.c_uint32, [C.c_uint32, C.c_uint32, C.c_uint32]),
diff --git a/cuda-pathtracer_amd/render.py b/cuda-pathtracer_amd/render.py
--- a/cuda-pathtracer_amd/render.py
+++ b/cuda-pathtracer_amd/render.py
@@ -160,6 +160,11 @@
     def last_restart_deferred(self) -> bool:
         out = C.c_int32(0)
         N.check(self._lib.ptamd_last_restart_deferred(self._h, C.byref(out)))
+        return out.value != 0
+
+    def last_restart_tight(self) -> bool:
+        out = C.c_int32(0)
+        N.check(self._lib.ptamd_last_restart_tight(self._h, C.byref(out)))
         return out.value != 0
 
     def scene_is_flat(self, scene_id: int, cubemap_id: int) -> bool:
diff --git a/include/ptamd.h b/include/ptamd.h
--- a/include/ptamd.h
+++ b/include/ptamd.h
@@ -443,6 +443,7 @@
 int ptamd_scene_cull_count(ptamd_context* ctx, uint32_t scene_id, uint32_t* out);
 int ptamd_last_restart_form(ptamd_context* ctx, int32_t* out);
 int ptamd_last_restart_deferred(ptamd_context* ctx, int32_t* out);
+int ptamd_last_restart_tight(ptamd_context* ctx, int32_t* out);
 int ptamd_host_skip_trace(const ptamd_face* faces, const ptamd_face* faces_refit, uint32_t n_faces, uint32_t mode, float threshold,
                           const uint8_t* skip_in, const float* rays, uint32_t n, int32_t* out, uint64_t* counters,
                           uint32_t* n_nodes, uint8_t* skip_out, uint32_t* words_out);
```
